# mpkuse/rgbd_odometry

Measured on NVIDIA B200. Metric: frame-pairs aligned/s (640x480, 4-lvl), higher is better.
Workload: dtype f32+f64

## Files before the change

rgbd_odometry_b200/csrc/capi.cu:

```cuda
#include <math.h>
#include <stdarg.h>
#include <stdlib.h>

#include <algorithm>
#include <new>
#include <vector>

#include "common.cuh"

static thread_local char g_err[512] = "";

void dvo_set_error(const char* fmt, ...) {
    va_list ap; va_start(ap, fmt); vsnprintf(g_err, sizeof(g_err), fmt, ap); va_end(ap);
}

static int level_dim(int dim, int level) { return (int)nearbyint((double)dim * ldexp(1.0, -level)); }

namespace {
struct StageTimer {
    dvo_ctx* c; int stage; bool on;
    StageTimer(dvo_ctx* c_, int s) : c(c_), stage(s), on(c_->timing) { if (on) cudaEventRecord(c->ev_a, c->stream); }
    ~StageTimer() {
        if (!on) return;
        cudaEventRecord(c->ev_b, c->stream); cudaEventSynchronize(c->ev_b);
        float ms = 0.f; cudaEventElapsedTime(&ms, c->ev_a, c->ev_b); c->stage_ms[stage] += ms;
    }
};
template <typename T> int dalloc(T** p, size_t n) {
    if (n == 0) { *p = nullptr; return DVO_OK; }
    cudaError_t e = cudaMalloc((void**)p, n * sizeof(T));
    if (e != cudaSuccess) { dvo_set_error("cudaMalloc(%zu bytes) failed: %s", n * sizeof(T), cudaGetErrorString(e)); return DVO_ERR_NOMEM; }
    return DVO_OK;
}
bool range_ok(dvo_ctx* c, int first, int count) { return c && first >= 0 && count >= 0 && first + count <= c->cfg.max_batch; }
int join_aux(dvo_ctx* c) {
    if (!c || !c->aux_pending) return DVO_OK;
    c->aux_pending = false;
    for (int k = 0; k < 2; ++k) DVO_CUDA(cudaStreamWaitEvent(c->stream, c->ev_aux_done[k], 0));
    return DVO_OK;
}
}

extern "C" {

const char* dvo_last_error(void) { return g_err; }

int dvo_device_count(void) {
    int n = 0;
    if (cudaGetDeviceCount(&n) != cudaSuccess) { cudaGetLastError(); return 0; }
    return n;
}

#define CREATE_CUDA(call)                                                                       \
    do {                                                                                        \
        cudaError_t e__ = (call);                                                               \
        if (e__ != cudaSuccess) {                                                               \
            dvo_set_error("%s:%d: %s -> %s", __FILE__, __LINE__, #call, cudaGetErrorString(e__)); \
            dvo_destroy(c);                                                                     \
            return DVO_ERR_CUDA;                                                                \
        }                                                                                       \
    } while (0)

int dvo_create(const dvo_config* cfg, dvo_ctx** out) {
    if (!cfg || !out) { dvo_set_error("dvo_create: null argument"); return DVO_ERR_ARG; }
    if (cfg->width < 8 || cfg->height < 8 || cfg->levels < 1 || cfg->levels > DVO_MAX_LEVELS || cfg->max_batch < 1 || cfg->max_batch > 65535 ||
        cfg->width >= DVO_EDT_INF_1D || cfg->height >= DVO_EDT_INF_1D) {
        dvo_set_error("dvo_create: bad config %dx%d levels=%d max_batch=%d", cfg->width, cfg->height, cfg->levels, cfg->max_batch);
        return DVO_ERR_ARG;
    }
    int ndev = 0;
    cudaError_t e = cudaGetDeviceCount(&ndev);
    if (e != cudaSuccess || ndev == 0) {
        dvo_set_error("dvo_create: no usable CUDA device (%s); this library has no CPU fallback", cudaGetErrorString(e));
        cudaGetLastError();
        return DVO_ERR_CUDA;
    }
    if (cfg->device < 0 || cfg->device >= ndev) { dvo_set_error("dvo_create: device %d out of range (%d devices)", cfg->device, ndev); return DVO_ERR_ARG; }
    DVO_CUDA(cudaSetDevice(cfg->device));
    if (const char* e = getenv("DVO_L2_FETCH")) { cudaDeviceSetLimit(cudaLimitMaxL2FetchGranularity, (size_t)atoi(e)); cudaGetLastError(); }
    dvo_ctx* c = new (std::nothrow) dvo_ctx();
    if (!c) return DVO_ERR_NOMEM;
    memset(c, 0, sizeof(*c));
    c->cfg = *cfg;
    PyrGeom& g = c->geom;
    g.L = cfg->levels; g.Bmax = cfg->max_batch;
    long long acc = 0; int maxP = 0;
    for (int l = 0; l < g.L; ++l) {
        g.w[l] = level_dim(cfg->width, l); g.h[l] = level_dim(cfg->height, l);
        if (g.w[l] < 2 || g.h[l] < 2) { dvo_set_error("dvo_create: level %d is %dx%d (too small)", l, g.w[l], g.h[l]); dvo_destroy(c); return DVO_ERR_ARG; }
        g.P[l] = g.w[l] * g.h[l]; g.off[l] = acc * g.Bmax; acc += g.P[l];
        if (g.P[l] > maxP) maxP = g.P[l];
    }
    g.total = acc * g.Bmax;
    long long acct = 0;
    for (int l = 0; l < g.L; ++l) {
        g.tw[l] = (g.w[l] + 3) >> 2; g.Pt[l] = g.tw[l] * ((g.h[l] + 3) >> 2) * 16;
        g.offt[l] = acct * g.Bmax; acct += g.Pt[l];
    }
    g.total_t = acct * g.Bmax;
    cudaDeviceProp prop;
    CREATE_CUDA(cudaGetDeviceProperties(&prop, cfg->device));
    c->sm_count = prop.multiProcessorCount;
    c->smem_optin = prop.sharedMemPerBlockOptin;
    c->solve_shape = (cfg->max_batch <= c->sm_count) ? 512 : 256;
    if (const char* e = getenv("DVO_SOLVE_SHAPE")) { const int v = atoi(e); if (v == 256 || v == 512) c->solve_shape = v; }
    c->texel_mode = 1;
    c->edt_band = 0;
    if (const char* e = getenv("DVO_EDT_BAND")) c->edt_band = atoi(e);
    if (const char* e = getenv("DVO_TEXEL_MODE")) c->texel_mode = atoi(e) ? 1 : 0;
    CREATE_CUDA(cudaStreamCreateWithFlags(&c->own_stream, cudaStreamNonBlocking));
    c->stream = c->own_stream;
    CREATE_CUDA(cudaStreamCreateWithFlags(&c->copy_stream, cudaStreamNonBlocking));
    for (int i = 0; i < 16; ++i) CREATE_CUDA(cudaEventCreateWithFlags(&c->ev_chunk[i], cudaEventDisableTiming));
    CREATE_CUDA(cudaEventCreateWithFlags(&c->ev_entry, cudaEventDisableTiming));
    for (int k = 0; k < 2; ++k) {
        CREATE_CUDA(cudaStreamCreateWithFlags(&c->aux[k], cudaStreamNonBlocking));
        CREATE_CUDA(cudaEventCreateWithFlags(&c->ev_pre[k], cudaEventDisableTiming));
        CREATE_CUDA(cudaEventCreateWithFlags(&c->ev_aux_done[k], cudaEventDisableTiming));
    }
    CREATE_CUDA(cudaEventCreateWithFlags(&c->ev_fork, cudaEventDisableTiming));
    c->e2e_chunk = 128;
    if (const char* e = getenv("DVO_E2E_CHUNK")) { const int v = atoi(e); if (v > 0) c->e2e_chunk = v; }
    CREATE_CUDA(cudaEventCreate(&c->ev_a));
    CREATE_CUDA(cudaEventCreate(&c->ev_b));

    const size_t T = (size_t)g.total, B = (size_t)g.Bmax;
    int rc = DVO_OK;
    auto A = [&](int r) { if (rc == DVO_OK) rc = r; };
    for (int f = 0; f < 2; ++f) { A(dalloc(&c->gray[f], T)); A(dalloc(&c->edge[f], T)); }
    A(dalloc(&c->depth[0], T));
    if (cfg->keep_now_depth) { A(dalloc(&c->depth[1], T)); A(dalloc(&c->prev_gray, B * (size_t)g.P[0])); A(dalloc(&c->prev_depth, B * (size_t)g.P[0])); }
    c->now_valid = (unsigned char*)calloc(B, 1); c->prev_valid = (unsigned char*)calloc(B, 1);
    A(dalloc(&c->gcol, T)); A(dalloc(&c->d2, T));
    if (c->texel_mode) A(dalloc(&c->tex8, (size_t)g.total_t)); else A(dalloc(&c->texel, T));
    A(dalloc(&c->ptsX, T)); A(dalloc(&c->ptsY, T)); A(dalloc(&c->ptsZ, T)); A(dalloc(&c->ptsPix, T));
    A(dalloc(&c->npts, B * g.L)); A(dalloc(&c->solve_order, B)); A(dalloc(&c->seq_mask, B)); A(dalloc(&c->seq_state, B)); A(dalloc(&c->nedge, 2 * B * g.L)); A(dalloc(&c->maxd2, B * g.L));
    A(dalloc(&c->pose0, B * 12)); A(dalloc(&c->pose, B * 12)); A(dalloc(&c->info, B));
    if (cfg->trace_iters > 0) A(dalloc(&c->trace, B * g.L * cfg->trace_iters * DVO_TRACE_DOUBLES));
    A(dalloc(&c->energy, B * g.L * DVO_ENERGY_ITERS));
    canny_scratch_layout(g, c->bm_off, c->bm_words, &c->bitmap_scratch_words);
    A(dalloc(&c->bitmap_scratch, c->bitmap_scratch_words * B * 2));
    if (rc != DVO_OK) { dvo_destroy(c); return rc; }
    CREATE_CUDA(cudaMemsetAsync(c->npts, 0, sizeof(int) * B * g.L, c->stream));
    CREATE_CUDA(cudaMemsetAsync(c->bitmap_scratch, 0, sizeof(uint32_t) * c->bitmap_scratch_words * B * 2, c->stream));
    CREATE_CUDA(cudaMemsetAsync(c->nedge, 0, sizeof(unsigned) * 2 * B * g.L, c->stream));
    CREATE_CUDA(cudaMemsetAsync(c->maxd2, 0, sizeof(unsigned) * B * g.L, c->stream));
    CREATE_CUDA(cudaMemsetAsync(c->info, 0, sizeof(dvo_pair_info) * B, c->stream));
    CREATE_CUDA(cudaMallocHost((void**)&c->h_pose, sizeof(double) * 12 * B));
    CREATE_CUDA(cudaMallocHost((void**)&c->h_info, sizeof(dvo_pair_info) * B));
    dvo_set_initial_pose(c, 0, g.Bmax, nullptr, DVO_MEM_HOST);
    CREATE_CUDA(cudaStreamSynchronize(c->stream));
    *out = c;
    return DVO_OK;
}

int dvo_destroy(dvo_ctx* c) {
    if (!c) return DVO_OK;
    cudaSetDevice(c->cfg.device);
    if (c->own_stream) cudaStreamSynchronize(c->own_stream);
    for (int f = 0; f < 2; ++f) { cudaFree(c->gray[f]); cudaFree(c->depth[f]); cudaFree(c->edge[f]); }
    cudaFree(c->gcol); cudaFree(c->d2); cudaFree(c->texel); cudaFree(c->tex8); cudaFree(c->ptsX); cudaFree(c->ptsY); cudaFree(c->ptsZ); cudaFree(c->ptsPix);
    cudaFree(c->npts); cudaFree(c->solve_order); cudaFree(c->seq_mask); cudaFree(c->seq_state); cudaFree(c->nedge); cudaFree(c->maxd2); cudaFree(c->pose0); cudaFree(c->pose); cudaFree(c->info);
    cudaFree(c->seq_rel); cudaFree(c->seq_kind); cudaFree(c->seq_reason); cudaFree(c->seq_glob); cudaFree(c->seq_cov); cudaFree(c->seq_gcov);
    cudaFree(c->cov_buf); cudaFree(c->cov_info_buf);
    for (int k = 0; k < 2; ++k) {
        cudaFree(c->seq_stage_g[k]); cudaFree(c->seq_stage_d[k]);
        if (c->seq_ev_ready[k]) cudaEventDestroy(c->seq_ev_ready[k]);
        if (c->seq_ev_free[k]) cudaEventDestroy(c->seq_ev_free[k]);
    }
    cudaFree(c->trace); cudaFree(c->energy); cudaFree(c->bitmap_scratch); cudaFree(c->prev_gray); cudaFree(c->prev_depth); cudaFree(c->raw_bgr); cudaFree(c->raw_depth);
    free(c->now_valid); free(c->prev_valid);
    if (c->h_pose) cudaFreeHost(c->h_pose);
    if (c->h_info) cudaFreeHost(c->h_info);
    if (c->ev_a) cudaEventDestroy(c->ev_a);
    if (c->ev_b) cudaEventDestroy(c->ev_b);
    if (c->own_stream) cudaStreamDestroy(c->own_stream);
    for (int k = 0; k < 2; ++k) {
        if (c->aux[k]) { cudaStreamSynchronize(c->aux[k]); cudaStreamDestroy(c->aux[k]); }
        if (c->ev_pre[k]) cudaEventDestroy(c->ev_pre[k]);
        if (c->ev_aux_done[k]) cudaEventDestroy(c->ev_aux_done[k]);
    }
    if (c->ev_fork) cudaEventDestroy(c->ev_fork);
    if (c->copy_stream) cudaStreamDestroy(c->copy_stream);
    for (int i = 0; i < 16; ++i) if (c->ev_chunk[i]) cudaEventDestroy(c->ev_chunk[i]);
    if (c->ev_entry) cudaEventDestroy(c->ev_entry);
    delete c;
    return DVO_OK;
}

int dvo_set_stream(dvo_ctx* c, void* s) {
    if (!c) return DVO_ERR_ARG;
    { int rc = join_aux(c); if (rc) return rc; }
    c->stream = s ? (cudaStream_t)s : c->own_stream;
    return DVO_OK;
}

int dvo_synchronize(dvo_ctx* c) {
    if (!c) return DVO_ERR_ARG;
    { int rc = join_aux(c); if (rc) return rc; }
    DVO_CUDA(cudaStreamSynchronize(c->stream));
    return DVO_OK;
}

int dvo_set_intrinsics(dvo_ctx* c, float fx, float fy, float cx, float cy) {
    if (!c) return DVO_ERR_ARG;
    c->K.fx = fx; c->K.fy = fy; c->K.cx = cx; c->K.cy = cy; c->haveK = true;
    return DVO_OK;
}

}

static int begin_set_frames(dvo_ctx* c, const char* who, int frame, int first, int count, bool have_gray, bool have_depth) {
    if (!range_ok(c, first, count) || (frame != DVO_FRAME_REF && frame != DVO_FRAME_NOW) || !have_gray) { dvo_set_error("%s: bad argument", who); return DVO_ERR_ARG; }
    if (frame == DVO_FRAME_REF && !have_depth) { dvo_set_error("%s: the reference frame needs depth", who); return DVO_ERR_ARG; }
    bool rotate = false;
    if (frame == DVO_FRAME_NOW && c->prev_gray) {
        if (!have_depth) { dvo_set_error("%s: a context with keep_now_depth needs the now frame's depth", who); return DVO_ERR_ARG; }
        bool any = false, all = true;
        for (int i = first; i < first + count; ++i) { any |= c->now_valid[i] != 0; all &= c->now_valid[i] != 0; }
        if (any && !all) { dvo_set_error("%s: slots [%d,%d) mix first and subsequent now frames", who, first, first + count); return DVO_ERR_STATE; }
        rotate = all && count > 0;
    }
    const size_t P0 = c->geom.P[0];
    if (rotate) {
        DVO_CUDA(cudaMemcpyAsync(c->prev_gray + P0 * first, c->gray[1] + lvl_at(c->geom, 0, first), P0 * count, cudaMemcpyDeviceToDevice, c->stream));
        DVO_CUDA(cudaMemcpyAsync(c->prev_depth + P0 * first, c->depth[1] + lvl_at(c->geom, 0, first), P0 * count * 2, cudaMemcpyDeviceToDevice, c->stream));
        for (int i = first; i < first + count; ++i) c->prev_valid[i] = 1;
    }
    if (frame == DVO_FRAME_NOW) for (int i = first; i < first + count; ++i) c->now_valid[i] = 1;
    return DVO_OK;
}

extern "C" {

int dvo_set_frames(dvo_ctx* c, int frame, int first, int count, const uint8_t* gray, const uint16_t* depth, int mem) {
    if (c) { const int jr = join_aux(c); if (jr) return jr; }
    { const int rc = begin_set_frames(c, "dvo_set_frames", frame, first, count, gray != nullptr, depth != nullptr); if (rc) return rc; }
    StageTimer t(c, DVO_STAGE_H2D);
    const size_t P0 = c->geom.P[0];
    const cudaMemcpyKind k = mem == DVO_MEM_DEVICE ? cudaMemcpyDeviceToDevice : cudaMemcpyHostToDevice;
    DVO_CUDA(cudaMemcpyAsync(c->gray[frame] + lvl_at(c->geom, 0, first), gray, P0 * count, k, c->stream));
    if (depth && c->depth[frame])
        DVO_CUDA(cudaMemcpyAsync(c->depth[frame] + lvl_at(c->geom, 0, first), depth, P0 * count * sizeof(uint16_t), k, c->stream));
    return DVO_OK;
}

int dvo_set_frames_raw(dvo_ctx* c, int frame, int first, int count, const uint8_t* bgr, const float* depth_m, int mem) {
    if (c) { const int jr = join_aux(c); if (jr) return jr; }
    { const int rc = begin_set_frames(c, "dvo_set_frames_raw", frame, first, count, bgr != nullptr, depth_m != nullptr); if (rc) return rc; }
    if (count == 0) return DVO_OK;
    StageTimer t(c, DVO_STAGE_H2D);
    const size_t P0 = c->geom.P[0];
    const uint8_t* d_bgr = bgr; const float* d_dm = depth_m;
    if (mem != DVO_MEM_DEVICE) {
        if (c->raw_capacity < (size_t)count) {
            DVO_CUDA(cudaStreamSynchronize(c->stream));
            cudaFree(c->raw_bgr); cudaFree(c->raw_depth); c->raw_bgr = nullptr; c->raw_depth = nullptr; c->raw_capacity = 0;
            int rc = dalloc(&c->raw_bgr, (size_t)count * P0 * 3); if (rc) return rc;
            rc = dalloc(&c->raw_depth, (size_t)count * P0); if (rc) return rc;
            c->raw_capacity = (size_t)count;
        }
        DVO_CUDA(cudaMemcpyAsync(c->raw_bgr, bgr, P0 * count * 3, cudaMemcpyHostToDevice, c->stream));
        if (depth_m) DVO_CUDA(cudaMemcpyAsync(c->raw_depth, depth_m, P0 * count * sizeof(float), cudaMemcpyHostToDevice, c->stream));
        d_bgr = c->raw_bgr; d_dm = depth_m ? c->raw_depth : nullptr;
    }
    return launch_ingest_raw(c, frame, first, count, d_bgr, d_dm);
}

int dvo_promote_now_to_ref(dvo_ctx* c, int first, int count) {
    if (c) { const int jr = join_aux(c); if (jr) return jr; }
    if (!range_ok(c, first, count)) return DVO_ERR_ARG;
    return launch_promote(c, first, count);
}

int dvo_build_pyramids(dvo_ctx* c, int first, int count, int frames_mask) {
    if (c) { const int jr = join_aux(c); if (jr) return jr; }
    if (!range_ok(c, first, count)) { dvo_set_error("dvo_build_pyramids: bad range"); return DVO_ERR_ARG; }
    if (count == 0) return DVO_OK;
    StageTimer t(c, DVO_STAGE_PYRAMID);
    return launch_pyramid(c, first, count, frames_mask);
}

int dvo_prepare(dvo_ctx* c, int first, int count, int frames_mask) {
    if (c) { const int jr = join_aux(c); if (jr) return jr; }
    if (!range_ok(c, first, count)) { dvo_set_error("dvo_prepare: bad range"); return DVO_ERR_ARG; }
    if (!c->haveK) { dvo_set_error("dvo_prepare: intrinsics not set (SolveDVO asserts isCameraIntrinsicsAvailable)"); return DVO_ERR_STATE; }
    if (count == 0) return DVO_OK;
    int rc;
    { StageTimer t(c, DVO_STAGE_CANNY); rc = launch_canny(c, first, count, frames_mask); if (rc) return rc; }
    if (frames_mask & 2) {
        if (c->texel_mode && c->edt_band >= 0) {
            StageTimer t(c, DVO_STAGE_EDT_ROWS); rc = launch_edt_pack(c, first, count); if (rc) return rc;
        } else {
            { StageTimer t(c, DVO_STAGE_EDT_ROWS); rc = launch_edt_rows(c, first, count); if (rc) return rc; }
            { StageTimer t(c, DVO_STAGE_NORMGRAD); rc = c->texel_mode ? launch_pack(c, first, count) : launch_normgrad(c, first, count); if (rc) return rc; }
        }
    }
    return DVO_OK;
}

int dvo_set_initial_pose(dvo_ctx* c, int first, int count, const double* R9T3, int mem) {
    if (c) { const int jr = join_aux(c); if (jr) return jr; }
    if (!range_ok(c, first, count)) return DVO_ERR_ARG;
    if (R9T3) {
        DVO_CUDA(cudaMemcpyAsync(c->pose0 + 12 * (size_t)first, R9T3, sizeof(double) * 12 * count,
                                 mem == DVO_MEM_DEVICE ? cudaMemcpyDeviceToDevice : cudaMemcpyHostToDevice, c->stream));
        if (mem != DVO_MEM_DEVICE) DVO_CUDA(cudaStreamSynchronize(c->stream));
    } else {
        std::vector<double> id((size_t)12 * count, 0.0);
        for (int i = 0; i < count; ++i) { id[12 * (size_t)i] = 1.0; id[12 * (size_t)i + 4] = 1.0; id[12 * (size_t)i + 8] = 1.0; }
        DVO_CUDA(cudaMemcpyAsync(c->pose0 + 12 * (size_t)first, id.data(), sizeof(double) * 12 * count, cudaMemcpyHostToDevice, c->stream));
        DVO_CUDA(cudaStreamSynchronize(c->stream));
    }
    return DVO_OK;
}

int dvo_run(dvo_ctx* c, int first, int count, const dvo_solver_params* p) {
    if (c) { const int jr = join_aux(c); if (jr) return jr; }
    if (!range_ok(c, first, count) || !p) { dvo_set_error("dvo_run: bad argument"); return DVO_ERR_ARG; }
    if (!c->haveK) { dvo_set_error("dvo_run: intrinsics not set"); return DVO_ERR_STATE; }
    if (count == 0) return DVO_OK;
    StageTimer t(c, DVO_STAGE_SOLVE);
    return launch_solve(c, first, count, p);
}

static int process_range(dvo_ctx* c, int first, int count, const dvo_solver_params* p, cudaEvent_t pre_done) {
    int rc;
    if ((rc = launch_pyramid(c, first, count, 3))) return rc;
    if ((rc = launch_canny(c, first, count, 3))) return rc;
    if (c->texel_mode && c->edt_band >= 0) { if ((rc = launch_edt_pack(c, first, count))) return rc; }
    else {
        if ((rc = launch_edt_rows(c, first, count))) return rc;
        if ((rc = c->texel_mode ? launch_pack(c, first, count) : launch_normgrad(c, first, count))) return rc;
    }
    if (pre_done) DVO_CUDA(cudaEventRecord(pre_done, c->stream));
    return launch_solve(c, first, count, p);
}

int dvo_process(dvo_ctx* c, int first, int count, const dvo_solver_params* p, double* d_poses) {
    if (!range_ok(c, first, count) || !p) { dvo_set_error("dvo_process: bad argument"); return DVO_ERR_ARG; }
    if (!c->haveK) { dvo_set_error("dvo_process: intrinsics not set"); return DVO_ERR_STATE; }
    if (count == 0) return DVO_OK;
    if (c->timing || count < 4 * c->sm_count) {
        int rc = join_aux(c); if (rc) return rc;
        if ((rc = dvo_build_pyramids(c, first, count, 3))) return rc;
        if ((rc = dvo_prepare(c, first, count, 3))) return rc;
        if ((rc = dvo_run(c, first, count, p))) return rc;
        if (d_poses) DVO_CUDA(cudaMemcpyAsync(d_poses, c->pose + 12 * (size_t)first, sizeof(double) * 12 * count, cudaMemcpyDeviceToDevice, c->stream));
        return DVO_OK;
    }
    if (c->aux_pending && (c->proc_first != first || c->proc_count != count)) { const int rc = join_aux(c); if (rc) return rc; }
    c->proc_first = first; c->proc_count = count;
    DVO_CUDA(cudaEventRecord(c->ev_fork, c->stream));
    const cudaStream_t user = c->stream;
    const int n0 = count / 2;
    const int starts[2] = {first, first + n0}, counts[2] = {n0, count - n0};
    int rc = DVO_OK;
    for (int k = 0; k < 2 && rc == DVO_OK; ++k) {
        cudaError_t e = cudaStreamWaitEvent(c->aux[k], c->ev_fork, 0);
        if (e == cudaSuccess && k == 1) e = cudaStreamWaitEvent(c->aux[1], c->ev_pre[0], 0);
        if (e != cudaSuccess) { dvo_set_error("dvo_process: %s", cudaGetErrorString(e)); rc = DVO_ERR_CUDA; break; }
        c->stream = c->aux[k];
        rc = process_range(c, starts[k], counts[k], p, c->ev_pre[k]);
        if (rc == DVO_OK && d_poses && cudaMemcpyAsync(d_poses + 12 * (size_t)(starts[k] - first), c->pose + 12 * (size_t)starts[k], sizeof(double) * 12 * counts[k],
                                                       cudaMemcpyDeviceToDevice, c->aux[k]) != cudaSuccess) rc = DVO_ERR_CUDA;
        if (rc == DVO_OK && cudaEventRecord(c->ev_aux_done[k], c->aux[k]) != cudaSuccess) rc = DVO_ERR_CUDA;
    }
    c->stream = user;
    c->aux_pending = true;
    if (rc != DVO_OK) join_aux(c);
    return rc;
}

int dvo_join(dvo_ctx* c) {
    if (!c) return DVO_ERR_ARG;
    return join_aux(c);
}

int dvo_join_stream(dvo_ctx* c, void* s) {
    if (!c) return DVO_ERR_ARG;
    if (!c->aux_pending) return DVO_OK;
    for (int k = 0; k < 2; ++k) DVO_CUDA(cudaStreamWaitEvent((cudaStream_t)s, c->ev_aux_done[k], 0));
    return DVO_OK;
}

int dvo_get_poses(dvo_ctx* c, int first, int count, double* R9T3, dvo_pair_info* info, int mem) {
    if (c) { const int jr = join_aux(c); if (jr) return jr; }
    if (!range_ok(c, first, count)) return DVO_ERR_ARG;
    StageTimer t(c, DVO_STAGE_D2H);
    const cudaMemcpyKind k = mem == DVO_MEM_DEVICE ? cudaMemcpyDeviceToDevice : cudaMemcpyDeviceToHost;
    if (R9T3) DVO_CUDA(cudaMemcpyAsync(R9T3, c->pose + 12 * (size_t)first, sizeof(double) * 12 * count, k, c->stream));
    if (info) DVO_CUDA(cudaMemcpyAsync(info, c->info + first, sizeof(dvo_pair_info) * count, k, c->stream));
    if (mem != DVO_MEM_DEVICE) DVO_CUDA(cudaStreamSynchronize(c->stream));
    return DVO_OK;
}

int dvo_align_batch(dvo_ctx* c, int count, const uint8_t* ref_gray, const uint16_t* ref_depth, const uint8_t* now_gray,
                    const uint16_t* now_depth, const dvo_solver_params* p, double* R9T3, dvo_pair_info* info) {
    if (c) { const int jr = join_aux(c); if (jr) return jr; }
    if (!c || count < 0 || !ref_gray || !ref_depth || !now_gray || !p) { dvo_set_error("dvo_align_batch: bad argument"); return DVO_ERR_ARG; }
    if (!c->haveK) { dvo_set_error("dvo_align_batch: intrinsics not set"); return DVO_ERR_STATE; }
    const size_t P0 = c->geom.P[0];
    const int B = c->cfg.max_batch;
    const bool timing = c->timing;
    c->timing = false;
    int rc = DVO_OK;
    for (int done = 0; done < count && rc == DVO_OK; done += B) {
        const int n = (count - done < B) ? count - done : B;
        if ((rc = dvo_set_initial_pose(c, 0, n, nullptr, DVO_MEM_HOST))) break;
        cudaError_t e = cudaEventRecord(c->ev_entry, c->stream);
        if (e == cudaSuccess) e = cudaStreamWaitEvent(c->copy_stream, c->ev_entry, 0);
        if (e != cudaSuccess) { dvo_set_error("dvo_align_batch: %s", cudaGetErrorString(e)); rc = DVO_ERR_CUDA; break; }
        int nchunks = (n + c->e2e_chunk - 1) / c->e2e_chunk;
        if (nchunks > 16) nchunks = 16;
        const int chunk = (n + nchunks - 1) / nchunks;
        int k = 0;
        for (int c0 = 0; c0 < n && rc == DVO_OK; c0 += chunk, ++k) {
            const int m = (n - c0 < chunk) ? n - c0 : chunk;
            const size_t src = P0 * (size_t)(done + c0);
            const long long dst = lvl_at(c->geom, 0, c0);
            e = cudaMemcpyAsync(c->gray[0] + dst, ref_gray + src, P0 * m, cudaMemcpyHostToDevice, c->copy_stream);
            if (e == cudaSuccess) e = cudaMemcpyAsync(c->depth[0] + dst, ref_depth + src, P0 * m * 2, cudaMemcpyHostToDevice, c->copy_stream);
            if (e == cudaSuccess) e = cudaMemcpyAsync(c->gray[1] + dst, now_gray + src, P0 * m, cudaMemcpyHostToDevice, c->copy_stream);
            if (e == cudaSuccess && now_depth && c->depth[1])
                e = cudaMemcpyAsync(c->depth[1] + dst, now_depth + src, P0 * m * 2, cudaMemcpyHostToDevice, c->copy_stream);
            if (e == cudaSuccess) e = cudaEventRecord(c->ev_chunk[k], c->copy_stream);
            if (e == cudaSuccess) e = cudaStreamWaitEvent(c->stream, c->ev_chunk[k], 0);
            if (e != cudaSuccess) { dvo_set_error("dvo_align_batch: %s", cudaGetErrorString(e)); rc = DVO_ERR_CUDA; break; }
            if ((rc = dvo_build_pyramids(c, c0, m, 3))) break;
            if ((rc = dvo_prepare(c, c0, m, 3))) break;
            if ((rc = dvo_run(c, c0, m, p))) break;
        }
        if (rc == DVO_OK)
            rc = dvo_get_poses(c, 0, n, R9T3 ? R9T3 + 12 * (size_t)done : nullptr, info ? info + done : nullptr, DVO_MEM_HOST);
    }
    c->timing = timing;
    return rc;
}

}

namespace {
__global__ void seq_gate_kernel(int nseq, int nframes, int t, dvo_keyframe_policy pol, int finest, const dvo_pair_info* __restrict__ info,
                                const double* __restrict__ pose, double* __restrict__ pose0, int* __restrict__ lastRef,
                                unsigned char* __restrict__ mask, double* __restrict__ rel, int* __restrict__ kind, int* __restrict__ reason) {
    const int s = blockIdx.x * blockDim.x + threadIdx.x;
    if (s >= nseq) return;
    const dvo_pair_info& I = info[s];
    int signal = 0, why = 0;
    if (pol.use_quality_gates) {
        if (I.laplacian_b > pol.laplacian_thresh) { signal = 1; why = 2; }
        if (I.visible_ratio[finest] < pol.visible_ratio_thresh) { signal = 1; why = 3; }
        if (I.npts[finest] < pol.min_reprojections) { signal = 1; why = 4; }
    }
    if (pol.keyframe_every > 0 && (t - lastRef[s]) == pol.keyframe_every) { signal = 1; why = 5; }
    const long long cur = (long long)s * nframes + t;
    if (signal && lastRef[s] != t - 1) {
        mask[s] = 1; lastRef[s] = t - 1;
        kind[cur - 1] = 2; reason[cur - 1] = why;
        for (int k = 0; k < 12; ++k) pose0[12 * (long long)s + k] = (k == 0 || k == 4 || k == 8) ? 1.0 : 0.0;
    } else {
        mask[s] = 0;
        for (int k = 0; k < 12; ++k) { const double v = pose[12 * (long long)s + k]; rel[12 * cur + k] = v; pose0[12 * (long long)s + k] = v; }
        kind[cur] = 0; reason[cur] = 0;
    }
}
__global__ void seq_finish_kernel(int nseq, int nframes, int t, const unsigned char* __restrict__ mask, const double* __restrict__ pose,
                                  double* __restrict__ pose0, double* __restrict__ rel, int* __restrict__ kind, int* __restrict__ reason) {
    const int s = blockIdx.x * blockDim.x + threadIdx.x;
    if (s >= nseq || !mask[s]) return;
    const long long cur = (long long)s * nframes + t;
    for (int k = 0; k < 12; ++k) { const double v = pose[12 * (long long)s + k]; rel[12 * cur + k] = v; pose0[12 * (long long)s + k] = v; }
    kind[cur] = 0; reason[cur] = 0;
}
__global__ void seq_init_kernel(int nseq, int nframes, double* __restrict__ pose0, int* __restrict__ lastRef, double* __restrict__ rel,
                                int* __restrict__ kind, int* __restrict__ reason) {
    const int s = blockIdx.x * blockDim.x + threadIdx.x;
    if (s >= nseq) return;
    lastRef[s] = 0;
    for (int k = 0; k < 12; ++k) { const double v = (k == 0 || k == 4 || k == 8) ? 1.0 : 0.0; pose0[12 * (long long)s + k] = v; rel[12 * (long long)s * nframes + k] = v; }
    kind[(long long)s * nframes] = 1; reason[(long long)s * nframes] = 1;
}

int run_sequences_core(dvo_ctx* c, int nseq, int nframes, const uint8_t* gray, const uint16_t* depth, int mem, const dvo_solver_params* p,
                       const dvo_keyframe_policy* pol, double* rel_poses, int* kind, int* reason, double* global_poses,
                       double* rel_cov, double* global_cov) {
    const char* who = rel_cov ? "dvo_run_sequences_cov" : "dvo_run_sequences";
    if (c) { const int jr = join_aux(c); if (jr) return jr; }
    if (!c || nseq < 1 || nseq > c->cfg.max_batch || nframes < 1 || !gray || !depth || !p || !pol || !rel_poses || !kind || (global_cov && !rel_cov)) {
        dvo_set_error("%s: bad argument", who); return DVO_ERR_ARG;
    }
    if (!c->prev_gray) { dvo_set_error("%s: create the context with keep_now_depth = 1", who); return DVO_ERR_STATE; }
    if (!c->haveK) { dvo_set_error("%s: intrinsics not set", who); return DVO_ERR_STATE; }
    int finest = -1;
    for (int l = 0; l < c->geom.L; ++l) if (p->iters[l] > 0) { finest = l; break; }
    if (finest < 0) { dvo_set_error("%s: no level has iterations", who); return DVO_ERR_ARG; }
    const size_t P0 = c->geom.P[0], n = (size_t)nseq * nframes;
    const bool host_in = (mem != DVO_MEM_DEVICE);
    int rc = DVO_OK;
    auto fail = [&](cudaError_t e) { if (e != cudaSuccess && rc == DVO_OK) { dvo_set_error("%s: %s", who, cudaGetErrorString(e)); rc = DVO_ERR_CUDA; } return rc != DVO_OK; };

    if (c->seq_rec_n < n) {
        cudaFree(c->seq_rel); cudaFree(c->seq_kind); cudaFree(c->seq_reason); c->seq_rel = nullptr; c->seq_kind = nullptr; c->seq_reason = nullptr; c->seq_rec_n = 0;
        fail(cudaMalloc((void**)&c->seq_rel, sizeof(double) * 12 * n)); fail(cudaMalloc((void**)&c->seq_kind, sizeof(int) * n)); fail(cudaMalloc((void**)&c->seq_reason, sizeof(int) * n));
        if (rc == DVO_OK) c->seq_rec_n = n;
    }
    if (host_in && c->seq_stage_slots < (size_t)nseq) {
        for (int k = 0; k < 2; ++k) { cudaFree(c->seq_stage_g[k]); cudaFree(c->seq_stage_d[k]); c->seq_stage_g[k] = nullptr; c->seq_stage_d[k] = nullptr; }
        c->seq_stage_slots = 0;
        for (int k = 0; k < 2 && rc == DVO_OK; ++k) {
            fail(cudaMalloc((void**)&c->seq_stage_g[k], P0 * nseq)); fail(cudaMalloc((void**)&c->seq_stage_d[k], P0 * nseq * sizeof(uint16_t)));
            if (!c->seq_ev_ready[k]) fail(cudaEventCreateWithFlags(&c->seq_ev_ready[k], cudaEventDisableTiming));
            if (!c->seq_ev_free[k]) fail(cudaEventCreateWithFlags(&c->seq_ev_free[k], cudaEventDisableTiming));
        }
        if (rc == DVO_OK) c->seq_stage_slots = (size_t)nseq;
    }
    if (rel_cov && c->seq_cov_n < n) {
        cudaFree(c->seq_cov); c->seq_cov = nullptr; c->seq_cov_n = 0;
        if (!fail(cudaMalloc((void**)&c->seq_cov, sizeof(double) * 36 * n))) c->seq_cov_n = n;
    }
    if (rc != DVO_OK) return rc;
    double* d_rel = c->seq_rel; int* d_kind = c->seq_kind; int* d_reason = c->seq_reason; double* d_glob = nullptr;
    uint8_t* stage_g[2] = {c->seq_stage_g[0], c->seq_stage_g[1]}; uint16_t* stage_d[2] = {c->seq_stage_d[0], c->seq_stage_d[1]};
    cudaEvent_t ev_ready[2] = {c->seq_ev_ready[0], c->seq_ev_ready[1]}, ev_free[2] = {c->seq_ev_free[0], c->seq_ev_free[1]};
    fail(cudaMemsetAsync(d_rel, 0, sizeof(double) * 12 * n, c->stream));
    fail(cudaMemsetAsync(d_kind, 0, sizeof(int) * n, c->stream));
    fail(cudaMemsetAsync(d_reason, 0, sizeof(int) * n, c->stream));
    if (rel_cov) fail(cudaMemsetAsync(c->seq_cov, 0, sizeof(double) * 36 * n, c->stream));
    if (host_in) { fail(cudaEventRecord(c->ev_entry, c->stream)); fail(cudaStreamWaitEvent(c->copy_stream, c->ev_entry, 0)); }

    bool staged_before[2] = {false, false};
    auto upload = [&](int t) {
        if (!host_in || t >= nframes || rc != DVO_OK) return;
        const int k = t & 1;
        if (staged_before[k]) fail(cudaStreamWaitEvent(c->copy_stream, ev_free[k], 0));
        fail(cudaMemcpy2DAsync(stage_g[k], P0, gray + (size_t)t * P0, (size_t)nframes * P0, P0, nseq, cudaMemcpyHostToDevice, c->copy_stream));
        fail(cudaMemcpy2DAsync(stage_d[k], P0 * 2, depth + (size_t)t * P0, (size_t)nframes * P0 * 2, P0 * 2, nseq, cudaMemcpyHostToDevice, c->copy_stream));
        fail(cudaEventRecord(ev_ready[k], c->copy_stream));
        staged_before[k] = true;
    };
    auto ingest = [&](int frame, int t) {
        if (rc != DVO_OK) return;
        uint8_t* dg = c->gray[frame] + lvl_at(c->geom, 0, 0); uint16_t* dd = c->depth[frame] + lvl_at(c->geom, 0, 0);
        if (frame == DVO_FRAME_NOW && c->now_valid[0]) {
            if (rc == DVO_OK) rc = launch_copy_bytes(c, c->prev_gray, dg, P0 * nseq);
            if (rc == DVO_OK) rc = launch_copy_bytes(c, c->prev_depth, dd, P0 * nseq * 2);
            for (int s2 = 0; s2 < nseq; ++s2) c->prev_valid[s2] = 1;
        }
        if (frame == DVO_FRAME_NOW) for (int s2 = 0; s2 < nseq; ++s2) c->now_valid[s2] = 1;
        if (host_in) {
            const int k = t & 1;
            fail(cudaStreamWaitEvent(c->stream, ev_ready[k], 0));
            if (rc == DVO_OK) rc = launch_copy_bytes(c, dg, stage_g[k], P0 * nseq);
            if (rc == DVO_OK) rc = launch_copy_bytes(c, dd, stage_d[k], P0 * nseq * 2);
            fail(cudaEventRecord(ev_free[k], c->stream));
        } else {
            fail(cudaMemcpy2DAsync(dg, P0, gray + (size_t)t * P0, (size_t)nframes * P0, P0, nseq, cudaMemcpyDeviceToDevice, c->stream));
            fail(cudaMemcpy2DAsync(dd, P0 * 2, depth + (size_t)t * P0, (size_t)nframes * P0 * 2, P0 * 2, nseq, cudaMemcpyDeviceToDevice, c->stream));
        }
    };

    const int blk = (nseq + 127) / 128;
    const bool timing = c->timing;
    c->timing = false;
    for (int s2 = 0; s2 < nseq; ++s2) { c->now_valid[s2] = 0; c->prev_valid[s2] = 0; }
    upload(0); upload(1);
    ingest(DVO_FRAME_REF, 0);
    if (rc == DVO_OK) rc = dvo_build_pyramids(c, 0, nseq, 1);
    if (rc == DVO_OK) rc = dvo_prepare(c, 0, nseq, 1);
    if (rc == DVO_OK) { seq_init_kernel<<<blk, 128, 0, c->stream>>>(nseq, nframes, c->pose0, c->seq_state, d_rel, d_kind, d_reason); c->launches++; fail(cudaGetLastError()); }
    int host_last_ref = 0;
    for (int t = 1; t < nframes && rc == DVO_OK; ++t) {
        ingest(DVO_FRAME_NOW, t);
        upload(t + 1);
        if (rc != DVO_OK) break;
        if ((rc = dvo_build_pyramids(c, 0, nseq, 2))) break;
        if ((rc = dvo_prepare(c, 0, nseq, 2))) break;
        bool switch_pass = t >= 2, first_solve = true;
        if (!pol->use_quality_gates) {
            switch_pass = t >= 2 && pol->keyframe_every > 0 && (t - host_last_ref) == pol->keyframe_every && host_last_ref != t - 1;
            if (switch_pass) { host_last_ref = t - 1; first_solve = false; }
        }
        if (first_solve && (rc = dvo_run(c, 0, nseq, p))) break;
        seq_gate_kernel<<<blk, 128, 0, c->stream>>>(nseq, nframes, t, *pol, finest, c->info, c->pose, c->pose0, c->seq_state, c->seq_mask, d_rel, d_kind, d_reason);
        c->launches++;
        if (fail(cudaGetLastError())) break;
        if (switch_pass) {
            c->active = c->seq_mask;
            rc = dvo_promote_now_to_ref(c, 0, nseq);
            if (rc == DVO_OK) rc = dvo_build_pyramids(c, 0, nseq, 1);
            if (rc == DVO_OK) rc = dvo_prepare(c, 0, nseq, 1);
            if (rc == DVO_OK) rc = dvo_run(c, 0, nseq, p);
            c->active = nullptr;
            if (rc != DVO_OK) break;
            seq_finish_kernel<<<blk, 128, 0, c->stream>>>(nseq, nframes, t, c->seq_mask, c->pose, c->pose0, d_rel, d_kind, d_reason);
            c->launches++;
            if (fail(cudaGetLastError())) break;
        }
        if (rel_cov && (rc = launch_cov(c, 0, nseq, finest, p, c->seq_cov + 36 * (size_t)t, nullptr, nframes))) break;
    }
    c->active = nullptr;
    c->timing = timing;
    if (rc == DVO_OK && (global_poses || global_cov)) {
        if (c->seq_glob_n < n) {
            cudaFree(c->seq_glob); c->seq_glob = nullptr; c->seq_glob_n = 0;
            if (!fail(cudaMalloc((void**)&c->seq_glob, sizeof(double) * 19 * n))) c->seq_glob_n = n;
        }
        if (global_cov && rc == DVO_OK && c->seq_gcov_n < n) {
            cudaFree(c->seq_gcov); c->seq_gcov = nullptr; c->seq_gcov_n = 0;
            if (!fail(cudaMalloc((void**)&c->seq_gcov, sizeof(double) * 36 * n))) c->seq_gcov_n = n;
        }
        d_glob = c->seq_glob;
        if (rc == DVO_OK) {
            rc = launch_gop(c, nseq, nframes, d_kind, d_rel, d_glob, global_cov ? c->seq_cov : nullptr, global_cov ? c->seq_gcov : nullptr);
            if (rc == DVO_OK && global_poses) fail(cudaMemcpyAsync(global_poses, d_glob, sizeof(double) * 19 * n, cudaMemcpyDeviceToHost, c->stream));
            if (rc == DVO_OK && global_cov) fail(cudaMemcpyAsync(global_cov, c->seq_gcov, sizeof(double) * 36 * n, cudaMemcpyDeviceToHost, c->stream));
        }
    }
    if (rc == DVO_OK) {
        fail(cudaMemcpyAsync(rel_poses, d_rel, sizeof(double) * 12 * n, cudaMemcpyDeviceToHost, c->stream));
        fail(cudaMemcpyAsync(kind, d_kind, sizeof(int) * n, cudaMemcpyDeviceToHost, c->stream));
        if (reason) fail(cudaMemcpyAsync(reason, d_reason, sizeof(int) * n, cudaMemcpyDeviceToHost, c->stream));
        if (rel_cov) fail(cudaMemcpyAsync(rel_cov, c->seq_cov, sizeof(double) * 36 * n, cudaMemcpyDeviceToHost, c->stream));
    }
    cudaStreamSynchronize(c->copy_stream);
    if (cudaStreamSynchronize(c->stream) != cudaSuccess && rc == DVO_OK) { dvo_set_error("%s: %s", who, cudaGetErrorString(cudaGetLastError())); rc = DVO_ERR_CUDA; }
    return rc;
}
}

extern "C" {

int dvo_run_sequences(dvo_ctx* c, int nseq, int nframes, const uint8_t* gray, const uint16_t* depth, const dvo_solver_params* p,
                      int keyframe_every, double* rel_poses, int* kind, double* global_poses) {
    dvo_keyframe_policy pol; memset(&pol, 0, sizeof(pol));
    pol.keyframe_every = keyframe_every; pol.use_quality_gates = 0; pol.laplacian_thresh = 3.0f; pol.visible_ratio_thresh = 0.8f; pol.min_reprojections = 50;
    return run_sequences_core(c, nseq, nframes, gray, depth, DVO_MEM_HOST, p, &pol, rel_poses, kind, nullptr, global_poses, nullptr, nullptr);
}

int dvo_run_sequences_gated(dvo_ctx* c, int nseq, int nframes, const uint8_t* gray, const uint16_t* depth, const dvo_solver_params* p,
                            const dvo_keyframe_policy* pol, double* rel_poses, int* kind, int* reason, double* global_poses) {
    return run_sequences_core(c, nseq, nframes, gray, depth, DVO_MEM_HOST, p, pol, rel_poses, kind, reason, global_poses, nullptr, nullptr);
}

int dvo_run_sequences_mem(dvo_ctx* c, int nseq, int nframes, const uint8_t* gray, const uint16_t* depth, int mem, const dvo_solver_params* p,
                          const dvo_keyframe_policy* pol, double* rel_poses, int* kind, int* reason, double* global_poses) {
    return run_sequences_core(c, nseq, nframes, gray, depth, mem, p, pol, rel_poses, kind, reason, global_poses, nullptr, nullptr);
}

int dvo_run_sequences_cov(dvo_ctx* c, int nseq, int nframes, const uint8_t* gray, const uint16_t* depth, int mem, const dvo_solver_params* p,
                          const dvo_keyframe_policy* pol, double* rel_poses, int* kind, int* reason, double* global_poses, double* rel_cov,
                          double* global_cov) {
    if (!rel_cov) { dvo_set_error("dvo_run_sequences_cov: rel_cov is required"); return DVO_ERR_ARG; }
    return run_sequences_core(c, nseq, nframes, gray, depth, mem, p, pol, rel_poses, kind, reason, global_poses, rel_cov, global_cov);
}

int dvo_pose_covariance(dvo_ctx* c, int first, int count, const dvo_solver_params* p, int level, double* cov36, dvo_cov_info* info, int mem) {
    if (c) { const int jr = join_aux(c); if (jr) return jr; }
    if (!range_ok(c, first, count) || !p || !cov36 || (mem != DVO_MEM_HOST && mem != DVO_MEM_DEVICE) || level < -1 || level >= c->geom.L ||
        (p->residual != DVO_RESIDUAL_DT_FLOOR && p->residual != DVO_RESIDUAL_DT_INTERP)) {
        dvo_set_error("dvo_pose_covariance: bad argument"); return DVO_ERR_ARG;
    }
    if (!c->haveK) { dvo_set_error("dvo_pose_covariance: intrinsics not set"); return DVO_ERR_STATE; }
    if (level < 0) for (int l = 0; l < c->geom.L; ++l) if (p->iters[l] > 0) { level = l; break; }
    if (level < 0) { dvo_set_error("dvo_pose_covariance: level = -1 and no level has iterations"); return DVO_ERR_ARG; }
    if (count == 0) return DVO_OK;
    if (mem == DVO_MEM_DEVICE) return launch_cov(c, first, count, level, p, cov36, info, 1);
    if (c->cov_cap < (size_t)count) {
        DVO_CUDA(cudaStreamSynchronize(c->stream));
        cudaFree(c->cov_buf); cudaFree(c->cov_info_buf); c->cov_buf = nullptr; c->cov_info_buf = nullptr; c->cov_cap = 0;
        int rc = dalloc(&c->cov_buf, (size_t)count * 36); if (rc) return rc;
        rc = dalloc(&c->cov_info_buf, (size_t)count); if (rc) return rc;
        c->cov_cap = (size_t)count;
    }
    const int rc = launch_cov(c, first, count, level, p, c->cov_buf, c->cov_info_buf, 1);
    if (rc) return rc;
    DVO_CUDA(cudaMemcpyAsync(cov36, c->cov_buf, sizeof(double) * 36 * count, cudaMemcpyDeviceToHost, c->stream));
    if (info) DVO_CUDA(cudaMemcpyAsync(info, c->cov_info_buf, sizeof(dvo_cov_info) * count, cudaMemcpyDeviceToHost, c->stream));
    DVO_CUDA(cudaStreamSynchronize(c->stream));
    return DVO_OK;
}

int dvo_level_dims(dvo_ctx* c, int level, int* w, int* h) {
    if (!c || level < 0 || level >= c->geom.L) return DVO_ERR_ARG;
    if (w) *w = c->geom.w[level];
    if (h) *h = c->geom.h[level];
    return DVO_OK;
}

int dvo_get_level_buffer(dvo_ctx* c, int slot, int frame, int level, int which, void* dst, size_t bytes) {
    if (c) { const int jr = join_aux(c); if (jr) return jr; }
    if (!range_ok(c, slot, 1) || level < 0 || level >= c->geom.L || (frame != 0 && frame != 1) || !dst) { dvo_set_error("dvo_get_level_buffer: bad argument"); return DVO_ERR_ARG; }
    const size_t P = c->geom.P[level];
    const long long o = lvl_at(c->geom, level, slot);
    const void* src = nullptr; size_t es = 0;
    switch (which) {
        case DVO_BUF_GRAY: src = c->gray[frame] + o; es = 1; break;
        case DVO_BUF_DEPTH: if (!c->depth[frame]) { dvo_set_error("depth not stored for this frame"); return DVO_ERR_STATE; } src = c->depth[frame] + o; es = 2; break;
        case DVO_BUF_EDGE: src = c->edge[frame] + o; es = 1; break;
        case DVO_BUF_D2: if (frame != DVO_FRAME_NOW) { dvo_set_error("d2 exists for the now frame only"); return DVO_ERR_ARG; } src = c->d2 + o; es = 4; break;
        case DVO_BUF_DTN: case DVO_BUF_GX: case DVO_BUF_GY:
            if (frame != DVO_FRAME_NOW) { dvo_set_error("DT exists for the now frame only"); return DVO_ERR_ARG; } src = c->texel ? c->texel + o : nullptr; es = 16; break;
        default: dvo_set_error("dvo_get_level_buffer: unknown buffer %d", which); return DVO_ERR_ARG;
    }
    if (which == DVO_BUF_D2 && c->texel_mode && c->edt_band >= 0) {
        if (bytes < P * 4) { dvo_set_error("dvo_get_level_buffer: destination too small"); return DVO_ERR_ARG; }
        int32_t* d_tmp = nullptr;
        DVO_CUDA(cudaMalloc((void**)&d_tmp, P * 4));
        const int rc = launch_d2_from_texels(c, slot, level, d_tmp);
        cudaError_t ce = rc ? cudaSuccess : cudaMemcpyAsync(dst, d_tmp, P * 4, cudaMemcpyDeviceToHost, c->stream);
        if (ce == cudaSuccess) ce = cudaStreamSynchronize(c->stream);
        cudaFree(d_tmp);
        if (rc) return rc;
        DVO_CUDA(ce);
        return DVO_OK;
    }
    if (which >= DVO_BUF_DTN) {
        if (bytes < P * 4) { dvo_set_error("dvo_get_level_buffer: destination too small"); return DVO_ERR_ARG; }
        std::vector<float> tmp(P * 4);
        float4* d_tmp = nullptr;
        if (!src) {
            DVO_CUDA(cudaMalloc((void**)&d_tmp, P * 16));
            const int rc = c->texel_mode ? launch_resolve_texels(c, slot, level, d_tmp) : launch_normgrad_into(c, slot, level, d_tmp);
            if (rc) { cudaFree(d_tmp); return rc; }
            src = d_tmp;
        }
        cudaError_t ce = cudaMemcpyAsync(tmp.data(), src, P * 16, cudaMemcpyDeviceToHost, c->stream);
        if (ce == cudaSuccess) ce = cudaStreamSynchronize(c->stream);
        cudaFree(d_tmp);
        DVO_CUDA(ce);
        const int comp = which - DVO_BUF_DTN;
        float* d = (float*)dst;
        for (size_t i = 0; i < P; ++i) d[i] = tmp[4 * i + comp];
        return DVO_OK;
    }
    if (bytes < P * es) { dvo_set_error("dvo_get_level_buffer: destination too small"); return DVO_ERR_ARG; }
    DVO_CUDA(cudaMemcpyAsync(dst, src, P * es, cudaMemcpyDeviceToHost, c->stream));
    DVO_CUDA(cudaStreamSynchronize(c->stream));
    if (which == DVO_BUF_DEPTH && level == 0) {
        uint16_t* d = (uint16_t*)dst;
        for (size_t i = 0; i < P; ++i) if (d[i] == 0) d[i] = 1;
    }
    return DVO_OK;
}

static int reference_order(dvo_ctx* c, int slot, int level, int n, std::vector<int>& perm) {
    perm.resize(n);
    if (n == 0) return DVO_OK;
    std::vector<int> pix(n);
    DVO_CUDA(cudaMemcpyAsync(pix.data(), c->ptsPix + lvl_at(c->geom, level, slot), sizeof(int) * n, cudaMemcpyDeviceToHost, c->stream));
    DVO_CUDA(cudaStreamSynchronize(c->stream));
    const int w = c->geom.w[level], h = c->geom.h[level];
    std::vector<long long> key(n);
    for (int i = 0; i < n; ++i) { const int y = pix[i] / w, x = pix[i] - y * w; key[i] = ((long long)x * h + y) * (long long)n + i; }
    std::sort(key.begin(), key.end());
    for (int k = 0; k < n; ++k) perm[k] = (int)(key[k] % n);
    return DVO_OK;
}

int dvo_get_points(dvo_ctx* c, int slot, int level, float* X, float* Y, float* Z, int capacity, int* n) {
    if (c) { const int jr = join_aux(c); if (jr) return jr; }
    if (!range_ok(c, slot, 1) || level < 0 || level >= c->geom.L || !n) return DVO_ERR_ARG;
    int cnt = 0;
    DVO_CUDA(cudaMemcpyAsync(&cnt, c->npts + (size_t)slot * c->geom.L + level, sizeof(int), cudaMemcpyDeviceToHost, c->stream));
    DVO_CUDA(cudaStreamSynchronize(c->stream));
    *n = cnt;
    const int m = cnt < capacity ? cnt : capacity;
    if (m <= 0 || !(X || Y || Z)) return DVO_OK;
    std::vector<int> perm;
    int rc = reference_order(c, slot, level, cnt, perm);
    if (rc) return rc;
    const long long o = lvl_at(c->geom, level, slot);
    std::vector<float> tmp(cnt);
    float* dst[3] = {X, Y, Z}; const float* src[3] = {c->ptsX + o, c->ptsY + o, c->ptsZ + o};
    for (int a = 0; a < 3; ++a) {
        if (!dst[a]) continue;
        DVO_CUDA(cudaMemcpyAsync(tmp.data(), src[a], sizeof(float) * cnt, cudaMemcpyDeviceToHost, c->stream));
        DVO_CUDA(cudaStreamSynchronize(c->stream));
        for (int k = 0; k < m; ++k) dst[a][k] = tmp[perm[k]];
    }
    return DVO_OK;
}

int dvo_eval_normal_equations(dvo_ctx* c, int slot, int level, const double* R9T3, int jacobian, int weight, int arithmetic,
                              float huber_k, double* H36, double* g6, double* sumsq, int* nvis, float* eps, float* w, float* u,
                              float* v, float* J) {
    dvo_solver_params prm;
    memset(&prm, 0, sizeof(prm));
    prm.jacobian = jacobian; prm.weight = weight; prm.arithmetic = arithmetic; prm.huber_k = huber_k;
    return dvo_eval_normal_equations_ex(c, slot, level, R9T3, &prm, H36, g6, sumsq, nvis, eps, w, u, v, J);
}

int dvo_eval_normal_equations_ex(dvo_ctx* c, int slot, int level, const double* R9T3, const dvo_solver_params* prm,
                                 double* H36, double* g6, double* sumsq, int* nvis, float* eps, float* w, float* u, float* v, float* J) {
    if (c) { const int jr = join_aux(c); if (jr) return jr; }
    if (!prm) return DVO_ERR_ARG;
    if (!range_ok(c, slot, 1) || level < 0 || level >= c->geom.L || !R9T3) return DVO_ERR_ARG;
    if (!c->haveK) { dvo_set_error("intrinsics not set"); return DVO_ERR_STATE; }
    int N = 0;
    DVO_CUDA(cudaMemcpyAsync(&N, c->npts + (size_t)slot * c->geom.L + level, sizeof(int), cudaMemcpyDeviceToHost, c->stream));
    DVO_CUDA(cudaStreamSynchronize(c->stream));
    double* d_pose = nullptr; double* d_out = nullptr; float* d_pp = nullptr;
    const bool pp = eps || w || u || v || J;
    const size_t n1 = (size_t)(N > 0 ? N : 1);
    {
        cudaError_t e = cudaMalloc((void**)&d_pose, sizeof(double) * 12);
        if (e == cudaSuccess) e = cudaMalloc((void**)&d_out, sizeof(double) * 44);
        if (e == cudaSuccess && pp) e = cudaMalloc((void**)&d_pp, sizeof(float) * n1 * 10);
        if (e == cudaSuccess) e = cudaMemcpyAsync(d_pose, R9T3, sizeof(double) * 12, cudaMemcpyHostToDevice, c->stream);
        if (e != cudaSuccess) {
            dvo_set_error("dvo_eval_normal_equations: %s", cudaGetErrorString(e));
            cudaFree(d_pose); cudaFree(d_out); cudaFree(d_pp);
            return DVO_ERR_CUDA;
        }
    }
    float *de = nullptr, *dw = nullptr, *du = nullptr, *dv = nullptr, *dJ = nullptr;
    if (pp) { de = d_pp; dw = d_pp + n1; du = d_pp + 2 * n1; dv = d_pp + 3 * n1; dJ = d_pp + 4 * n1; }
    int rc = launch_eval(c, slot, level, d_pose, prm->jacobian, prm->weight, prm->arithmetic, prm->huber_k, prm->residual, d_out, de, dw, du, dv, dJ);
    if (rc == DVO_OK) {
        double out[44];
        std::vector<float> host(pp ? n1 * 10 : 0);
        cudaError_t e = cudaMemcpyAsync(out, d_out, sizeof(out), cudaMemcpyDeviceToHost, c->stream);
        if (e == cudaSuccess && pp && N > 0) e = cudaMemcpyAsync(host.data(), d_pp, sizeof(float) * n1 * 10, cudaMemcpyDeviceToHost, c->stream);
        if (e == cudaSuccess) e = cudaStreamSynchronize(c->stream);
        if (e != cudaSuccess) { dvo_set_error("dvo_eval_normal_equations: %s", cudaGetErrorString(e)); rc = DVO_ERR_CUDA; }
        else {
            if (g6) memcpy(g6, out, sizeof(double) * 6);
            if (H36) memcpy(H36, out + 6, sizeof(double) * 36);
            if (sumsq) *sumsq = out[42];
            if (nvis) *nvis = (int)out[43];
            if (pp && N > 0) {
                std::vector<int> perm;
                rc = reference_order(c, slot, level, N, perm);
                if (rc == DVO_OK)
                    for (int k = 0; k < N; ++k) {
                        const size_t i = (size_t)perm[k];
                        if (eps) eps[k] = host[i];
                        if (w) w[k] = host[n1 + i];
                        if (u) u[k] = host[2 * n1 + i];
                        if (v) v[k] = host[3 * n1 + i];
                        if (J) for (int q = 0; q < 6; ++q) J[6 * (size_t)k + q] = host[4 * n1 + 6 * i + q];
                    }
            }
        }
    }
    cudaFree(d_pose); cudaFree(d_out); cudaFree(d_pp);
    return rc;
}

int dvo_get_trace(dvo_ctx* c, int slot, int level, double* trace) {
    if (c) { const int jr = join_aux(c); if (jr) return jr; }
    if (!range_ok(c, slot, 1) || level < 0 || level >= c->geom.L || !trace) return DVO_ERR_ARG;
    if (!c->trace) { dvo_set_error("dvo_get_trace: context created with trace_iters = 0"); return DVO_ERR_STATE; }
    const size_t n = (size_t)c->cfg.trace_iters * DVO_TRACE_DOUBLES;
    DVO_CUDA(cudaMemcpyAsync(trace, c->trace + ((size_t)slot * c->geom.L + level) * n, sizeof(double) * n, cudaMemcpyDeviceToHost, c->stream));
    DVO_CUDA(cudaStreamSynchronize(c->stream));
    return DVO_OK;
}

int dvo_get_energies(dvo_ctx* c, int slot, int level, float* energies, int capacity) {
    if (c) { const int jr = join_aux(c); if (jr) return jr; }
    if (!range_ok(c, slot, 1) || level < 0 || level >= c->geom.L || !energies || capacity < 0) return DVO_ERR_ARG;
    const int n = capacity < DVO_ENERGY_ITERS ? capacity : DVO_ENERGY_ITERS;
    if (n == 0) return DVO_OK;
    DVO_CUDA(cudaMemcpyAsync(energies, c->energy + ((size_t)slot * c->geom.L + level) * DVO_ENERGY_ITERS, sizeof(float) * n, cudaMemcpyDeviceToHost, c->stream));
    DVO_CUDA(cudaStreamSynchronize(c->stream));
    return DVO_OK;
}

int dvo_enable_timing(dvo_ctx* c, int on) {
    if (!c) return DVO_ERR_ARG;
    c->timing = on != 0;
    for (int i = 0; i < DVO_STAGE_COUNT; ++i) c->stage_ms[i] = 0.f;
    return DVO_OK;
}

int dvo_get_stage_ms(dvo_ctx* c, float* ms) {
    if (!c || !ms) return DVO_ERR_ARG;
    for (int i = 0; i < DVO_STAGE_COUNT; ++i) { ms[i] = c->stage_ms[i]; c->stage_ms[i] = 0.f; }
    return DVO_OK;
}

long long dvo_launch_count(dvo_ctx* c) { return c ? c->launches : 0; }

int dvo_gop_compose(dvo_ctx* c, int nseq, int nframes, const int* kind, const double* rel, double* out, int mem) {
    if (c) { const int jr = join_aux(c); if (jr) return jr; }
    if (!c || nseq < 1 || nframes < 1 || !kind || !rel || !out) return DVO_ERR_ARG;
    const size_t n = (size_t)nseq * nframes;
    if (mem == DVO_MEM_DEVICE) return launch_gop(c, nseq, nframes, kind, rel, out, nullptr, nullptr);
    int* d_kind = nullptr; double* d_rel = nullptr; double* d_out = nullptr;
    {
        cudaError_t e = cudaMalloc((void**)&d_kind, sizeof(int) * n);
        if (e == cudaSuccess) e = cudaMalloc((void**)&d_rel, sizeof(double) * 12 * n);
        if (e == cudaSuccess) e = cudaMalloc((void**)&d_out, sizeof(double) * 19 * n);
        if (e == cudaSuccess) e = cudaMemcpyAsync(d_kind, kind, sizeof(int) * n, cudaMemcpyHostToDevice, c->stream);
        if (e == cudaSuccess) e = cudaMemcpyAsync(d_rel, rel, sizeof(double) * 12 * n, cudaMemcpyHostToDevice, c->stream);
        if (e != cudaSuccess) {
            dvo_set_error("dvo_gop_compose: %s", cudaGetErrorString(e));
            cudaFree(d_kind); cudaFree(d_rel); cudaFree(d_out);
            return DVO_ERR_CUDA;
        }
    }
    int rc = launch_gop(c, nseq, nframes, d_kind, d_rel, d_out, nullptr, nullptr);
    if (rc == DVO_OK) {
        cudaError_t e = cudaMemcpyAsync(out, d_out, sizeof(double) * 19 * n, cudaMemcpyDeviceToHost, c->stream);
        if (e == cudaSuccess) e = cudaStreamSynchronize(c->stream);
        if (e != cudaSuccess) { dvo_set_error("dvo_gop_compose: %s", cudaGetErrorString(e)); rc = DVO_ERR_CUDA; }
    }
    cudaFree(d_kind); cudaFree(d_rel); cudaFree(d_out);
    return rc;
}

struct dvo_blob { void* d; size_t bytes; int device; };

int dvo_blob_create(size_t bytes, int device, dvo_blob** out) {
    if (!out || bytes == 0) { dvo_set_error("dvo_blob_create: bad argument"); return DVO_ERR_ARG; }
    int ndev = 0;
    if (cudaGetDeviceCount(&ndev) != cudaSuccess || ndev < 1) { cudaGetLastError(); dvo_set_error("dvo_blob_create: no usable CUDA device (there is no CPU fallback)"); return DVO_ERR_CUDA; }
    if (device < 0 || device >= ndev) { dvo_set_error("dvo_blob_create: device %d out of range", device); return DVO_ERR_ARG; }
    DVO_CUDA(cudaSetDevice(device));
    dvo_blob* b = new (std::nothrow) dvo_blob();
    if (!b) return DVO_ERR_NOMEM;
    b->bytes = bytes; b->device = device; b->d = nullptr;
    if (cudaMalloc(&b->d, bytes) != cudaSuccess) { cudaGetLastError(); delete b; dvo_set_error("dvo_blob_create: cudaMalloc(%zu) failed", bytes); return DVO_ERR_NOMEM; }
    *out = b;
    return DVO_OK;
}
int dvo_blob_upload(dvo_blob* b, const void* host_src, size_t bytes) {
    if (!b || !host_src || bytes > b->bytes) { dvo_set_error("dvo_blob_upload: bad argument"); return DVO_ERR_ARG; }
    DVO_CUDA(cudaSetDevice(b->device));
    DVO_CUDA(cudaMemcpy(b->d, host_src, bytes, cudaMemcpyHostToDevice));
    return DVO_OK;
}
int dvo_blob_download(dvo_blob* b, void* host_dst, size_t bytes) {
    if (!b || !host_dst || bytes > b->bytes) { dvo_set_error("dvo_blob_download: bad argument"); return DVO_ERR_ARG; }
    DVO_CUDA(cudaSetDevice(b->device));
    DVO_CUDA(cudaMemcpy(host_dst, b->d, bytes, cudaMemcpyDeviceToHost));
    return DVO_OK;
}
void* dvo_blob_device_ptr(dvo_blob* b) { return b ? b->d : nullptr; }
size_t dvo_blob_bytes(dvo_blob* b) { return b ? b->bytes : 0; }
int dvo_blob_destroy(dvo_blob* b) {
    if (!b) return DVO_OK;
    cudaSetDevice(b->device);
    cudaFree(b->d);
    delete b;
    return DVO_OK;
}

}
```

rgbd_odometry_b200/csrc/common.cuh:

```cuda
#pragma once
#include <cuda_runtime.h>
#include <stdint.h>
#include <stdio.h>
#include <string.h>

#include "../../include/dvo_b200.h"

#define DVO_EDT_INF_1D 16384
#define DVO_EDT_INF (1 << 28)

struct PyrGeom {
    int L, Bmax;
    int w[DVO_MAX_LEVELS], h[DVO_MAX_LEVELS], P[DVO_MAX_LEVELS];
    long long off[DVO_MAX_LEVELS];
    long long total;
    int tw[DVO_MAX_LEVELS], Pt[DVO_MAX_LEVELS];
    long long offt[DVO_MAX_LEVELS];
    long long total_t;
};
__host__ __device__ inline long long lvl_at(const PyrGeom& g, int l, int b) { return g.off[l] + (long long)b * g.P[l]; }
__host__ __device__ inline long long tex_at(const PyrGeom& g, int l, int b) { return g.offt[l] + (long long)b * g.Pt[l]; }

#define DVO_TEX_ESCAPE 0x80000000u
__host__ __device__ inline int tex_index(int x, int y, int tw) {
    return (((y >> 2) * tw + (x >> 2)) << 4) | ((y & 2) << 2) | ((x & 2) << 1) | ((y & 1) << 1) | (x & 1);
}

struct Intr { float fx, fy, cx, cy; };

#define DVO_TRACE_DOUBLES 56
#define DVO_ENERGY_ITERS 128

struct dvo_ctx {
    dvo_config cfg;
    PyrGeom geom;
    Intr K;
    bool haveK;
    cudaStream_t own_stream, stream, copy_stream;
    cudaEvent_t ev_chunk[16], ev_entry;
    cudaStream_t aux[2];
    cudaEvent_t ev_fork, ev_pre[2], ev_aux_done[2];
    bool aux_pending;
    int proc_first, proc_count;
    int e2e_chunk;
    uint8_t* seq_stage_g[2]; uint16_t* seq_stage_d[2]; size_t seq_stage_slots;
    cudaEvent_t seq_ev_ready[2], seq_ev_free[2];
    double* seq_rel; int* seq_kind; int* seq_reason; double* seq_glob; size_t seq_rec_n, seq_glob_n;
    double* seq_cov; double* seq_gcov; size_t seq_cov_n, seq_gcov_n;
    double* cov_buf; dvo_cov_info* cov_info_buf; size_t cov_cap;
    int sm_count;
    int solve_shape;
    size_t smem_optin;

    uint8_t* gray[2];
    uint16_t* depth[2];
    uint8_t* prev_gray;
    uint16_t* prev_depth;
    unsigned char* now_valid;
    unsigned char* prev_valid;
    uint8_t* edge[2];
    uint16_t* gcol;
    int32_t* d2;
    float4* texel;
    uint2* tex8;
    int edt_band;
    int texel_mode;
    float *ptsX, *ptsY, *ptsZ;
    int* ptsPix;
    int* npts;
    int* solve_order;
    unsigned char* seq_mask;
    const unsigned char* active;
    int* seq_state;
    unsigned* nedge;
    unsigned* maxd2;
    double* pose0;
    double* pose;
    dvo_pair_info* info;
    double* trace;
    float* energy;
    uint32_t* bitmap_scratch;
    size_t bitmap_scratch_words;
    long long bm_off[DVO_MAX_LEVELS];
    int bm_words[DVO_MAX_LEVELS];
    size_t canny_smem_optin;

    uint8_t* raw_bgr; float* raw_depth; size_t raw_capacity;

    double* h_pose;
    dvo_pair_info* h_info;

    bool timing;
    cudaEvent_t ev_a, ev_b;
    float stage_ms[DVO_STAGE_COUNT];
    long long launches;
};

void dvo_set_error(const char* fmt, ...);

#define DVO_CUDA(call)                                                                          \
    do {                                                                                        \
        cudaError_t e__ = (call);                                                               \
        if (e__ != cudaSuccess) {                                                               \
            dvo_set_error("%s:%d: %s -> %s", __FILE__, __LINE__, #call, cudaGetErrorString(e__)); \
            return DVO_ERR_CUDA;                                                                \
        }                                                                                       \
    } while (0)

int launch_pyramid(dvo_ctx* c, int first, int count, int frames_mask);
int launch_canny(dvo_ctx* c, int first, int count, int frames_mask);
void canny_scratch_layout(const PyrGeom& g, long long* bm_off, int* bm_words, size_t* words_per_image);
int launch_edt_rows(dvo_ctx* c, int first, int count);
int launch_normgrad(dvo_ctx* c, int first, int count);
int launch_pack(dvo_ctx* c, int first, int count);
int launch_edt_pack(dvo_ctx* c, int first, int count);
int launch_d2_from_texels(dvo_ctx* c, int slot, int level, int32_t* d_out);
int launch_normgrad_into(dvo_ctx* c, int slot, int level, float4* d_out);
int launch_resolve_texels(dvo_ctx* c, int slot, int level, float4* d_out);
int launch_solve(dvo_ctx* c, int first, int count, const dvo_solver_params* p);
int launch_eval(dvo_ctx* c, int slot, int level, const double* d_pose12, int jac, int weight, int arith, float huber_k, int residual,
                double* d_out , float* d_eps, float* d_w, float* d_u, float* d_v, float* d_J);
int launch_cov(dvo_ctx* c, int first, int count, int level, const dvo_solver_params* p, double* d_cov, dvo_cov_info* d_info, long long stride);
int launch_gop(dvo_ctx* c, int nseq, int nframes, const int* d_kind, const double* d_rel, double* d_out, const double* d_rel_cov, double* d_glob_cov);
int launch_promote(dvo_ctx* c, int first, int count);
int launch_ingest_raw(dvo_ctx* c, int frame, int first, int count, const uint8_t* d_bgr, const float* d_depth_m);
int launch_copy_bytes(dvo_ctx* c, void* dst, const void* src, size_t n);

template <int ARITH> struct Ar;
template <> struct Ar<DVO_ARITH_EXACT> {
    static __device__ __forceinline__ float mul(float a, float b) { return __fmul_rn(a, b); }
    static __device__ __forceinline__ float add(float a, float b) { return __fadd_rn(a, b); }
    static __device__ __forceinline__ float sub(float a, float b) { return __fsub_rn(a, b); }
    static __device__ __forceinline__ float div(float a, float b) { return __fdiv_rn(a, b); }
    static __device__ __forceinline__ float dot2(float a, float b, float c, float d) { return __fadd_rn(__fmul_rn(a, b), __fmul_rn(c, d)); }
    static __device__ __forceinline__ float dot3(float a, float b, float c, float d, float e, float f) {
        return __fadd_rn(__fadd_rn(__fmul_rn(a, b), __fmul_rn(c, d)), __fmul_rn(e, f));
    }
    static __device__ __forceinline__ float diff2(float a, float b, float c, float d) { return __fsub_rn(__fmul_rn(a, b), __fmul_rn(c, d)); }
    static __device__ __forceinline__ float weight_ref(float r) {
        float rr = __fmul_rn(r, r);
        return __double2float_rn(__ddiv_rn(6.0, __dadd_rn(6.0, __dmul_rn((double)rr, 4.0))));
    }
};
template <> struct Ar<DVO_ARITH_FAST> {
    static __device__ __forceinline__ float mul(float a, float b) { return a * b; }
    static __device__ __forceinline__ float add(float a, float b) { return a + b; }
    static __device__ __forceinline__ float sub(float a, float b) { return a - b; }
    static __device__ __forceinline__ float div(float a, float b) { return __fdividef(a, b); }
    static __device__ __forceinline__ float dot2(float a, float b, float c, float d) { return fmaf(c, d, a * b); }
    static __device__ __forceinline__ float dot3(float a, float b, float c, float d, float e, float f) { return fmaf(e, f, fmaf(c, d, a * b)); }
    static __device__ __forceinline__ float diff2(float a, float b, float c, float d) { return fmaf(a, b, -(c * d)); }
    static __device__ __forceinline__ float weight_ref(float r) { return __fdividef(1.5f, fmaf(r, r, 1.5f)); }
};
```

rgbd_odometry_b200/csrc/preprocess.cu:

```cuda
#include <stdlib.h>

#include "common.cuh"

struct PyrArgs {
    PyrGeom g;
    uint8_t* gray;
    uint16_t* depth;
    int first;
    int sub_total;
    int l0;
    const unsigned char* active;
};

__global__ void __launch_bounds__(256) pyramid_nearest_kernel(PyrArgs a) {
    const int b = a.first + blockIdx.y;
    if (a.active && !a.active[b]) return;
    int q = blockIdx.x * blockDim.x + threadIdx.x;
    if (q >= a.sub_total) return;
    int l = a.l0;
    while (l < a.g.L - 1 && q >= a.g.P[l]) { q -= a.g.P[l]; ++l; }
    const int w = a.g.w[l], W0 = a.g.w[0], H0 = a.g.h[0];
    const int y = q / w, x = q - y * w;
    const int sy = min(y << l, H0 - 1), sx = min(x << l, W0 - 1);
    const long long src = lvl_at(a.g, 0, b) + (long long)sy * W0 + sx;
    const long long dst = lvl_at(a.g, l, b) + q;
    a.gray[dst] = a.gray[src];
    if (a.depth) { uint16_t d = a.depth[src]; a.depth[dst] = d == 0 ? (uint16_t)1 : d; }
}

__global__ void __launch_bounds__(256) pyramid_level1_vec4_kernel(PyrArgs a) {
    const int b = a.first + blockIdx.y;
    if (a.active && !a.active[b]) return;
    const int w1 = a.g.w[1], W0 = a.g.w[0], H0 = a.g.h[0];
    const int q4 = blockIdx.x * blockDim.x + threadIdx.x;
    if (q4 * 4 >= a.g.P[1]) return;
    const int y = (q4 * 4) / w1, x = q4 * 4 - y * w1;
    const int sy = min(2 * y, H0 - 1);
    const long long src = lvl_at(a.g, 0, b) + (long long)sy * W0 + 2 * x;
    const long long dst = lvl_at(a.g, 1, b) + (long long)q4 * 4;
    const uint2 gv = *reinterpret_cast<const uint2*>(a.gray + src);
    const uint32_t gout = (gv.x & 0xFFu) | ((gv.x >> 8) & 0xFF00u) | ((gv.y & 0xFFu) << 16) | ((gv.y << 8) & 0xFF000000u);
    *reinterpret_cast<uint32_t*>(a.gray + dst) = gout;
    if (a.depth) {
        const uint4 dv = *reinterpret_cast<const uint4*>(a.depth + src);
        uint32_t d0 = dv.x & 0xFFFFu, d1 = dv.y & 0xFFFFu, d2 = dv.z & 0xFFFFu, d3 = dv.w & 0xFFFFu;
        d0 = d0 ? d0 : 1u; d1 = d1 ? d1 : 1u; d2 = d2 ? d2 : 1u; d3 = d3 ? d3 : 1u;
        *reinterpret_cast<uint2*>(a.depth + dst) = make_uint2(d0 | (d1 << 16), d2 | (d3 << 16));
    }
}

__global__ void __launch_bounds__(256) pyramid_level1_vec8_kernel(PyrArgs a) {
    const int b = a.first + blockIdx.y;
    if (a.active && !a.active[b]) return;
    const int w1 = a.g.w[1], W0 = a.g.w[0], H0 = a.g.h[0];
    const int q8 = blockIdx.x * blockDim.x + threadIdx.x;
    if (q8 * 8 >= a.g.P[1]) return;
    const int y = (q8 * 8) / w1, x = q8 * 8 - y * w1;
    const int sy = min(2 * y, H0 - 1);
    const long long src = lvl_at(a.g, 0, b) + (long long)sy * W0 + 2 * x;
    const long long dst = lvl_at(a.g, 1, b) + (long long)q8 * 8;
    const uint4 gv = *reinterpret_cast<const uint4*>(a.gray + src);
    uint4 d0, d1;
    if (a.depth) { d0 = *reinterpret_cast<const uint4*>(a.depth + src); d1 = *reinterpret_cast<const uint4*>(a.depth + src + 8); }
    auto even_bytes = [](uint32_t lo, uint32_t hi) { return __byte_perm(lo, hi, 0x6420); };
    *reinterpret_cast<uint2*>(a.gray + dst) = make_uint2(even_bytes(gv.x, gv.y), even_bytes(gv.z, gv.w));
    if (a.depth) {
        auto fix = [](uint32_t v) { v &= 0xFFFFu; return v ? v : 1u; };
        *reinterpret_cast<uint4*>(a.depth + dst) = make_uint4(fix(d0.x) | (fix(d0.y) << 16), fix(d0.z) | (fix(d0.w) << 16),
                                                              fix(d1.x) | (fix(d1.y) << 16), fix(d1.z) | (fix(d1.w) << 16));
    }
}

__global__ void __launch_bounds__(256) pyramid_nearest_vec4_kernel(PyrArgs a) {
    const int b = a.first + blockIdx.y;
    if (a.active && !a.active[b]) return;
    int q = (blockIdx.x * blockDim.x + threadIdx.x) * 4;
    if (q >= a.sub_total) return;
    int l = a.l0;
    while (l < a.g.L - 1 && q >= a.g.P[l]) { q -= a.g.P[l]; ++l; }
    const int w = a.g.w[l], W0 = a.g.w[0], H0 = a.g.h[0];
    const int y = q / w, x = q - y * w;
    const int sy = min(y << l, H0 - 1);
    const long long row = lvl_at(a.g, 0, b) + (long long)sy * W0;
    const long long dst = lvl_at(a.g, l, b) + q;
    int sx[4];
#pragma unroll
    for (int j = 0; j < 4; ++j) sx[j] = min((x + j) << l, W0 - 1);
    uint32_t gv[4];
#pragma unroll
    for (int j = 0; j < 4; ++j) gv[j] = a.gray[row + sx[j]];
    if (a.depth) {
        uint32_t dv[4];
#pragma unroll
        for (int j = 0; j < 4; ++j) { dv[j] = a.depth[row + sx[j]]; }
#pragma unroll
        for (int j = 0; j < 4; ++j) dv[j] = dv[j] ? dv[j] : 1u;
        *reinterpret_cast<uint2*>(a.depth + dst) = make_uint2(dv[0] | (dv[1] << 16), dv[2] | (dv[3] << 16));
    }
    *reinterpret_cast<uint32_t*>(a.gray + dst) = gv[0] | (gv[1] << 8) | (gv[2] << 16) | (gv[3] << 24);
}

int launch_pyramid(dvo_ctx* c, int first, int count, int frames_mask) {
    const PyrGeom& g = c->geom;
    if (g.L < 2) return DVO_OK;
    const bool vec1 = (g.w[0] == 2 * g.w[1]) && (g.w[1] % 4 == 0);
    const int l0 = vec1 ? 2 : 1;
    int sub = 0;
    bool vec_rest = true;
    for (int l = l0; l < g.L; ++l) { sub += g.P[l]; vec_rest = vec_rest && (g.w[l] % 4 == 0) && (g.off[l] % 4 == 0) && (g.P[l] % 4 == 0); }
    for (int f = 0; f < 2; ++f) {
        if (!(frames_mask & (1 << f))) continue;
        PyrArgs a; a.g = g; a.gray = c->gray[f]; a.depth = c->depth[f]; a.first = first; a.sub_total = sub; a.l0 = l0; a.active = c->active;
        if (vec1 && g.w[1] % 8 == 0 && g.off[1] % 8 == 0 && g.P[1] % 8 == 0 && g.P[0] % 16 == 0) {
            dim3 grid1((g.P[1] / 8 + 255) / 256, count);
            pyramid_level1_vec8_kernel<<<grid1, 256, 0, c->stream>>>(a);
            c->launches++;
        } else if (vec1) {
            dim3 grid1((g.P[1] / 4 + 255) / 256, count);
            pyramid_level1_vec4_kernel<<<grid1, 256, 0, c->stream>>>(a);
            c->launches++;
        }
        if (sub > 0 && vec_rest) {
            dim3 grid((sub / 4 + 255) / 256, count);
            pyramid_nearest_vec4_kernel<<<grid, 256, 0, c->stream>>>(a);
            c->launches++;
        } else if (sub > 0) {
            dim3 grid((sub + 255) / 256, count);
            pyramid_nearest_kernel<<<grid, 256, 0, c->stream>>>(a);
            c->launches++;
        }
    }
    DVO_CUDA(cudaGetLastError());
    return DVO_OK;
}

struct CannyArgs {
    const uint8_t* gray[2];
    uint8_t* edge[2];
    const uint16_t* depth;
    uint16_t* gcol;
    float *X, *Y, *Z;
    int* pix;
    int* npts;
    unsigned* nedge[2];
    int w, h, P, L;
    int frame0;
    int count;
    long long gscratch_frame_stride;
    float tmpfx, tmpfy, tmpcx, tmpcy;
    uint32_t* gscratch;
    long long gscratch_stride;
    int first;
    int bm_words;
    const unsigned char* active;
};

__device__ __forceinline__ void sobel3(const uint8_t* __restrict__ g, int w, int h, int y, int x, int& dx, int& dy) {
    const int ym = max(y - 1, 0), yp = min(y + 1, h - 1), xm = max(x - 1, 0), xp = min(x + 1, w - 1);
    const uint8_t* r0 = g + ym * w; const uint8_t* r1 = g + y * w; const uint8_t* r2 = g + yp * w;
    const int a = r0[xm], b = r0[x], c = r0[xp], d = r1[xm], f = r1[xp], p = r2[xm], q = r2[x], r = r2[xp];
    dx = (c + 2 * f + r) - (a + 2 * d + p);
    dy = (p + 2 * q + r) - (a + 2 * b + c);
}
__device__ __forceinline__ int mag_at(const uint8_t* __restrict__ g, int w, int h, int y, int x) {
    if ((unsigned)y >= (unsigned)h || (unsigned)x >= (unsigned)w) return 0;
    int dx, dy; sobel3(g, w, h, y, x, dx, dy);
    return dx * dx + dy * dy;
}

__device__ __forceinline__ uint32_t expand4(uint32_t nib) { return (((nib & 0xFu) * 0x00204081u) & 0x01010101u) * 0xFFu; }

__device__ __forceinline__ void row_sums(const uint8_t* __restrict__ grow, int w, int x, int lane, int& hs, int& hb) {
    const int v = (x < w) ? (int)grow[x] : 0;
    int l = __shfl_up_sync(0xffffffffu, v, 1), r = __shfl_down_sync(0xffffffffu, v, 1);
    if (lane == 0) l = (x > 0 && x < w) ? (int)grow[x - 1] : v;
    if (lane == 31) r = (x + 1 < w) ? (int)grow[x + 1] : v;
    if (x + 1 >= w) r = v;
    hs = r - l; hb = l + 2 * v + r;
}

#ifndef DVO_NMS_L2_AHEAD
#define DVO_NMS_L2_AHEAD 4
#endif
#ifndef DVO_NMS_MIN_BLOCKS
#define DVO_NMS_MIN_BLOCKS 2
#endif
#ifndef DVO_NMS_ROWS
#define DVO_NMS_ROWS 48
#endif
#ifndef DVO_NMS_WARPS
#define DVO_NMS_WARPS 8
#endif
constexpr int NMS_ROWS = DVO_NMS_ROWS, NMS_WARPS = DVO_NMS_WARPS;
struct NmsArgs {
    const uint8_t* gray[2];
    uint32_t* scratch;
    long long slot_stride, frame_stride;
    long long off[DVO_MAX_LEVELS];
    long long bm_off[DVO_MAX_LEVELS];
    int w[DVO_MAX_LEVELS], h[DVO_MAX_LEVELS], P[DVO_MAX_LEVELS], bm_words[DVO_MAX_LEVELS];
    int chunks[DVO_MAX_LEVELS], strips[DVO_MAX_LEVELS], task_end[DVO_MAX_LEVELS];
    int L, first, count, frame0;
    float low, high;
    const unsigned char* active;
};
struct NmsSums { float s[4], b[4], sH, bH; };
struct NmsMags { float m[4], L, R; };
struct NmsGrad { float dx[4], dy[4]; };

template <bool VEC>
__global__ void __launch_bounds__(NMS_WARPS * 32, DVO_NMS_MIN_BLOCKS) sobel_nms_kernel(NmsArgs a) {
    const int lane = threadIdx.x & 31;
    int task = blockIdx.x * NMS_WARPS + (threadIdx.x >> 5);
    int l = 0;
    while (l < a.L && task >= a.task_end[l]) ++l;
    if (l >= a.L) return;
    if (l) task -= a.task_end[l - 1];
    const int chunks = a.chunks[l], strips = a.strips[l];
    const int chunk = task % chunks, t2 = task / chunks, strip = t2 % strips, img = t2 / strips;
    const int second = (img >= a.count) ? 1 : 0;
    const int frame = second ? DVO_FRAME_NOW : a.frame0;
    const int b = a.first + img - second * a.count;
    if (a.active && !a.active[b]) return;
    const int w = a.w[l], h = a.h[l];
    const int wd = (w + 31) >> 5, pitch = wd + 2;
    const uint8_t* __restrict__ g = a.gray[frame] + a.off[l] + (long long)b * a.P[l];
    uint32_t* Cb = a.scratch + (long long)b * a.slot_stride + (long long)frame * a.frame_stride + a.bm_off[l];
    const int bmw = a.bm_words[l];
    const int c0 = chunk << 7, xb = c0 + (lane << 2);
    const int y0 = strip * NMS_ROWS, y1 = min(h, y0 + NMS_ROWS);
    const bool first_lane = (lane == 0), last_lane = (lane == 31);
    const bool halo_valid = first_lane ? (c0 > 0) : (last_lane && c0 + 128 < w);
    const bool self_left = (xb == 0), self_right = (xb + 4 >= w);
    const int hx0 = first_lane ? c0 - 2 : c0 + 128;
    const uint32_t sel_near = 0x7440u + (first_lane ? 1u : 0u), sel_far = 0x7440u + (first_lane ? 0u : 1u);
    const float lowt = (xb < w) ? a.low : 3.0e38f, high = a.high;
    const float K = 13573.0f / 32768.0f;

    const bool in_image = (xb < w);
    const uint8_t* __restrict__ gx = g + (in_image ? xb : 0);
    const uint8_t* __restrict__ gh = g + (halo_valid ? hx0 : 0);
    const unsigned roff_max = (unsigned)((h - 1) * w);
    auto load_row = [&](unsigned roff, uint32_t& wv, uint32_t& hv) {
        if (VEC) {
            wv = in_image ? *reinterpret_cast<const uint32_t*>(gx + roff) : 0u;
            hv = halo_valid ? (uint32_t)*reinterpret_cast<const uint16_t*>(gh + roff) : 0u;
        } else {
            const uint8_t* __restrict__ row = g + roff;
            wv = 0u;
#pragma unroll
            for (int j = 0; j < 4; ++j) wv |= (uint32_t)row[min(xb + j, w - 1)] << (8 * j);
            hv = halo_valid ? ((uint32_t)row[hx0] | ((uint32_t)row[min(hx0 + 1, w - 1)] << 8)) : 0u;
        }
    };
    auto byte_f = [](uint32_t wv, uint32_t sel) { return __uint_as_float(__byte_perm(wv, 0x4B000000u, sel)) - 8388608.0f; };
    auto sums = [&](uint32_t wv, uint32_t hv, NmsSums& S) {
        float v[4];
#pragma unroll
        for (int j = 0; j < 4; ++j) v[j] = byte_f(wv, 0x7440u + j);
        const float hn = byte_f(hv, sel_near), hf = byte_f(hv, sel_far);
        float lft = __shfl_up_sync(0xffffffffu, v[3], 1), rgt = __shfl_down_sync(0xffffffffu, v[0], 1);
        if (first_lane) lft = hn;
        if (last_lane) rgt = hn;
        if (self_left) lft = v[0];
        if (self_right) rgt = v[3];
        S.s[0] = v[1] - lft;  S.s[1] = v[2] - v[0]; S.s[2] = v[3] - v[1]; S.s[3] = rgt - v[2];
        S.b[0] = fmaf(2.0f, v[0], lft) + v[1];  S.b[1] = fmaf(2.0f, v[1], v[0]) + v[2];
        S.b[2] = fmaf(2.0f, v[2], v[1]) + v[3]; S.b[3] = fmaf(2.0f, v[3], v[2]) + rgt;
        const float gm1 = first_lane ? hf : v[3], gp1 = first_lane ? v[0] : hf;
        S.sH = gp1 - gm1; S.bH = fmaf(2.0f, hn, gm1) + gp1;
    };
    auto grad_mag = [&](bool inside, const NmsSums& A, const NmsSums& B, const NmsSums& Cs, NmsGrad& G, NmsMags& M) {
        float mH;
        if (inside) {
#pragma unroll
            for (int j = 0; j < 4; ++j) {
                G.dx[j] = fmaf(2.0f, B.s[j], A.s[j]) + Cs.s[j]; G.dy[j] = Cs.b[j] - A.b[j];
                M.m[j] = fmaf(G.dx[j], G.dx[j], G.dy[j] * G.dy[j]);
            }
            const float dxH = fmaf(2.0f, B.sH, A.sH) + Cs.sH, dyH = Cs.bH - A.bH;
            mH = halo_valid ? fmaf(dxH, dxH, dyH * dyH) : 0.0f;
            if (!VEC) {
#pragma unroll
                for (int j = 0; j < 4; ++j) if (xb + j >= w) M.m[j] = 0.0f;
            }
        } else {
#pragma unroll
            for (int j = 0; j < 4; ++j) { G.dx[j] = 0.0f; G.dy[j] = 0.0f; M.m[j] = 0.0f; }
            mH = 0.0f;
        }
        M.L = __shfl_up_sync(0xffffffffu, M.m[3], 1); M.R = __shfl_down_sync(0xffffffffu, M.m[0], 1);
        if (first_lane) M.L = mH;
        if (last_lane) M.R = mH;
        if (self_right) M.R = 0.0f;
    };

    uint32_t wv, hv;
    NmsSums S0, S1, S2;
    NmsMags M0, M1, M2;
    NmsGrad G0, G1;
    auto row_off = [&](int r) { return min((unsigned)max(r, 0) * (unsigned)w, roff_max); };
    load_row(row_off(y0 - 2), wv, hv); sums(wv, hv, S0);
    load_row(row_off(y0 - 1), wv, hv); sums(wv, hv, S1);
    load_row(row_off(y0), wv, hv);     sums(wv, hv, S2);
    grad_mag(y0 > 0, S0, S1, S2, G0, M0);
    load_row(row_off(y0 + 1), wv, hv); sums(wv, hv, S0);
    grad_mag(true, S1, S2, S0, G0, M1);
    uint32_t wvn, hvn;
    load_row(row_off(y0 + 2), wvn, hvn);
    unsigned roff_next = row_off(y0 + 3);
    unsigned roff_l2 = row_off(y0 + 3 + DVO_NMS_L2_AHEAD);

    const int widx = (c0 >> 5) + (lane >> 3);
    const bool writer = ((lane & 7) == 0) && widx < wd;
    uint32_t* Cp = Cb + (long long)(y0 + 1) * pitch + 1 + widx;
    const int sh = (lane & 3) << 2;

    auto nms_row = [&](const NmsMags& P, const NmsMags& C, const NmsMags& N, const NmsGrad& Gc) {
        float crm[4], ncm[4];
#pragma unroll
        for (int j = 0; j < 4; ++j) { crm[j] = ((j < 3) ? C.m[j < 3 ? j + 1 : 3] : C.R) - 0.5f; ncm[j] = N.m[j] - 0.5f; }
        uint32_t bits = 0u;
#pragma unroll
        for (int j = 0; j < 4; ++j) {
            const float m = C.m[j];
            const float cl = j ? C.m[j > 0 ? j - 1 : 0] : C.L;
            const float pl = j ? P.m[j > 0 ? j - 1 : 0] : P.L, pr = (j < 3) ? P.m[j < 3 ? j + 1 : 3] : P.R;
            const float nl = j ? N.m[j > 0 ? j - 1 : 0] : N.L, nr = (j < 3) ? N.m[j < 3 ? j + 1 : 3] : N.R;
            const float adx = fabsf(Gc.dx[j]), ady = fabsf(Gc.dy[j]);
            const float t = adx * K, u = fmaf(adx, -2.0f, ady);
            const bool horiz = ady < t, vert = u > t;
            const bool neg = Gc.dx[j] * Gc.dy[j] < 0.0f;
            const float da = neg ? pr : pl, db = neg ? nl : nr;
            const float na = horiz ? cl : (vert ? P.m[j] : da);
            const float nb = horiz ? crm[j] : (vert ? ncm[j] : db);
            const bool cand = (m > na) && (m > nb) && (m > lowt);
            const bool strong = cand && (m > high);
            bits |= (cand ? (1u << j) : 0u) | (strong ? (0x10000u << j) : 0u);
        }
        bits <<= sh;
        bits |= __shfl_xor_sync(0xffffffffu, bits, 1);
        bits |= __shfl_xor_sync(0xffffffffu, bits, 2);
        const uint32_t hi = __shfl_down_sync(0xffffffffu, bits, 4);
        if (writer) {
            Cp[0] = __byte_perm(bits, hi, 0x5410);
            Cp[bmw] = __byte_perm(bits, hi, 0x7632);
        }
        Cp += pitch;
    };
    auto row_step = [&](const NmsSums& A, const NmsSums& B, NmsSums& Cs, const NmsMags& P, const NmsMags& C, NmsMags& N,
                        const NmsGrad& Gc, NmsGrad& Gn) {
        wv = wvn; hv = hvn;
        load_row(roff_next, wvn, hvn); roff_next = min(roff_next + (unsigned)w, roff_max);
        if (DVO_NMS_L2_AHEAD > 0) {
            if (in_image) asm volatile("prefetch.global.L2 [%0];" :: "l"(gx + roff_l2));
            roff_l2 = min(roff_l2 + (unsigned)w, roff_max);
        }
        sums(wv, hv, Cs);
        grad_mag(true, A, B, Cs, Gn, N);
        nms_row(P, C, N, Gc);
    };
    const int yend = (y1 == h) ? y1 - 1 : y1;
    int y = y0;
    for (; y + 6 <= yend; y += 6) {
        row_step(S2, S0, S1, M0, M1, M2, G0, G1);
        row_step(S0, S1, S2, M1, M2, M0, G1, G0);
        row_step(S1, S2, S0, M2, M0, M1, G0, G1);
        row_step(S2, S0, S1, M0, M1, M2, G1, G0);
        row_step(S0, S1, S2, M1, M2, M0, G0, G1);
        row_step(S1, S2, S0, M2, M0, M1, G1, G0);
    }
    for (; y < yend; ++y) {
        row_step(S2, S0, S1, M0, M1, M2, G0, G1);
        S2 = S0; S0 = S1; M0 = M1; M1 = M2; G0 = G1;
    }
    if (y1 == h) {
        grad_mag(false, S2, S0, S1, G1, M2);
        nms_row(M0, M1, M2, G0);
    }
}

constexpr int CANNY_MAX_WARPS = 24;
#ifndef DVO_CANNY_INTERLEAVE
#define DVO_CANNY_INTERLEAVE 1
#endif
#ifndef DVO_CANNY_STOP_AFTER
#define DVO_CANNY_STOP_AFTER 0
#endif

template <bool GLOBAL_BITMAPS> struct HystPtr { typedef volatile uint32_t* type; };
template <> struct HystPtr<true> { typedef uint32_t* type; };

template <bool GLOBAL_BITMAPS>
__global__ void __launch_bounds__(768, 2) canny_kernel(CannyArgs a) {
    extern __shared__ uint32_t smem_u32[];
    __shared__ int s_scan[CANNY_MAX_WARPS + 1];
    __shared__ int s_base;
    __shared__ unsigned s_cnt;
    __shared__ unsigned char s_chg[2][768];
    const int T = blockDim.x;
    const int tid = threadIdx.x, lane = tid & 31, warp = tid >> 5;
#if DVO_CANNY_INTERLEAVE
    const bool both = a.count != 0x7fffffff;
    const int second = both ? (int)(blockIdx.x & 1u) : 0;
    const int frame = second ? DVO_FRAME_NOW : a.frame0;
    const int b = a.first + (both ? (int)(blockIdx.x >> 1) : (int)blockIdx.x);
#else
    const int second = (blockIdx.x >= (unsigned)a.count) ? 1 : 0;
    const int frame = second ? DVO_FRAME_NOW : a.frame0;
    const int b = a.first + (int)blockIdx.x - second * a.count;
#endif
    const bool do_points = (frame == DVO_FRAME_REF), do_cols = (frame == DVO_FRAME_NOW);
    if (a.active && !a.active[b]) return;
    const int w = a.w, h = a.h;
    const int wd = (w + 31) >> 5, pitch = wd + 2;
    const int nwords = a.bm_words;
    uint32_t* C = GLOBAL_BITMAPS ? a.gscratch + (long long)b * a.gscratch_stride + (long long)frame * a.gscratch_frame_stride : smem_u32;
    uint32_t* E = C + nwords;

    if (GLOBAL_BITMAPS) {
        for (int i = tid; i < pitch; i += T) { C[i] = 0u; E[i] = 0u; C[(h + 1) * pitch + i] = 0u; E[(h + 1) * pitch + i] = 0u; }
        for (int y = tid; y < h; y += T) {
            C[(y + 1) * pitch] = 0u; E[(y + 1) * pitch] = 0u; C[(y + 1) * pitch + wd + 1] = 0u; E[(y + 1) * pitch + wd + 1] = 0u;
        }
    } else {
        const uint32_t* __restrict__ src = a.gscratch + (long long)b * a.gscratch_stride + (long long)frame * a.gscratch_frame_stride;
        if ((reinterpret_cast<uintptr_t>(src) & 15) == 0 && (nwords & 1) == 0) {
            const uint4* s4 = reinterpret_cast<const uint4*>(src); uint4* d4 = reinterpret_cast<uint4*>(C);
            for (int i = tid; i < (nwords >> 1); i += T) d4[i] = s4[i];
        } else {
            for (int i = tid; i < 2 * nwords; i += T) C[i] = src[i];
        }
    }
    if (tid == 0) { s_cnt = 0u; s_base = 0; }
    __syncthreads();

#if DVO_CANNY_STOP_AFTER == 1
    return;
#endif
    {
        const int Hs = max(1, min(h, min(T, 768) / wd));
        const int Rh = (h + Hs - 1) / Hs;
        const int items = wd * Hs;
        const int sh = tid / wd, wx = tid - sh * wd;
        const bool owner = tid < items;
        const int ya = sh * Rh, yb = min(h, ya + Rh);
        for (int i = tid; i < 2 * 768; i += T) (&s_chg[0][0])[i] = (i < 768) ? 1 : 0;
        __syncthreads();
        int cur = 0;
        for (;;) {
            int changed = 0;
            bool active = false;
            if (owner && ya < yb) {
                for (int dsy = -1; dsy <= 1 && !active; ++dsy)
                    for (int dwx = -1; dwx <= 1; ++dwx) {
                        const int s2 = sh + dsy, w2 = wx + dwx;
                        if (s2 >= 0 && s2 < Hs && w2 >= 0 && w2 < wd && s_chg[cur][s2 * wd + w2]) { active = true; break; }
                    }
            }
            if (active) {
                auto spread = [](uint32_t l, uint32_t c, uint32_t r) { return c | (c << 1) | (c >> 1) | (l >> 31) | (r << 31); };
                auto flood = [](uint32_t f, uint32_t c) {
                    const uint32_t up = ((c + f) ^ c) & c;
                    const uint32_t cr = __brev(c), fr = __brev(f);
                    return f | up | __brev(((cr + fr) ^ cr) & cr);
                };
                typename HystPtr<GLOBAL_BITMAPS>::type Ev = E;
                const uint32_t* Cv = C;
                {
                    int idx = (ya + 1) * pitch + wx + 1;
                    uint32_t sp = spread(Ev[idx - pitch - 1], Ev[idx - pitch], Ev[idx - pitch + 1]);
                    uint32_t el = Ev[idx - 1], ec = Ev[idx], er = Ev[idx + 1];
                    for (int y = ya; y < yb; ++y, idx += pitch) {
                        const uint32_t nl = Ev[idx + pitch - 1], nc = Ev[idx + pitch], nr = Ev[idx + pitch + 1];
                        const uint32_t c = Cv[idx];
                        uint32_t f = ec;
                        if (c != 0u && ec != c) {
                            f = flood(ec | (c & (sp | spread(el, ec, er) | spread(nl, nc, nr))), c);
                            if (f != ec) { Ev[idx] = f; changed = 1; }
                        }
                        sp = spread(el, f, er); el = nl; ec = nc; er = nr;
                    }
                }
                {
                    int idx = yb * pitch + wx + 1;
                    uint32_t sp = spread(Ev[idx + pitch - 1], Ev[idx + pitch], Ev[idx + pitch + 1]);
                    uint32_t el = Ev[idx - 1], ec = Ev[idx], er = Ev[idx + 1];
                    for (int y = yb - 1; y >= ya; --y, idx -= pitch) {
                        const uint32_t nl = Ev[idx - pitch - 1], nc = Ev[idx - pitch], nr = Ev[idx - pitch + 1];
                        const uint32_t c = Cv[idx];
                        uint32_t f = ec;
                        if (c != 0u && ec != c) {
                            f = flood(ec | (c & (sp | spread(el, ec, er) | spread(nl, nc, nr))), c);
                            if (f != ec) { Ev[idx] = f; changed = 1; }
                        }
                        sp = spread(el, f, er); el = nl; ec = nc; er = nr;
                    }
                }
            }
            if (owner) s_chg[cur ^ 1][tid] = (unsigned char)changed;
            cur ^= 1;
            if (!__syncthreads_or(changed)) break;
        }
    }

#if DVO_CANNY_STOP_AFTER == 2
    return;
#endif
    const int nw = h * wd;
    {
        uint8_t* eo = a.edge[frame] + (long long)b * a.P;
        unsigned cnt = 0;
        const bool vec_ok = (w % 16 == 0) && ((reinterpret_cast<uintptr_t>(eo) & 15) == 0);
        for (int q = tid; q < nw; q += T) {
            const int y = q / wd, wx = q - y * wd;
            const uint32_t e = E[(y + 1) * pitch + wx + 1];
            cnt += __popc(e);
            const int x0 = wx << 5;
            if (vec_ok && x0 + 32 <= w) {
                uint4 v0, v1;
                v0.x = expand4(e); v0.y = expand4(e >> 4); v0.z = expand4(e >> 8); v0.w = expand4(e >> 12);
                v1.x = expand4(e >> 16); v1.y = expand4(e >> 20); v1.z = expand4(e >> 24); v1.w = expand4(e >> 28);
                uint4* dst = reinterpret_cast<uint4*>(eo + (long long)y * w + x0);
                dst[0] = v0; dst[1] = v1;
            } else {
                for (int i = 0; i < 32 && x0 + i < w; ++i) eo[(long long)y * w + x0 + i] = ((e >> i) & 1u) ? 255 : 0;
            }
        }
        for (int o = 16; o > 0; o >>= 1) cnt += __shfl_down_sync(0xffffffffu, cnt, o);
        if (lane == 0 && cnt) atomicAdd(&s_cnt, cnt);
    }

#if DVO_CANNY_STOP_AFTER == 3
    return;
#endif
    if (do_points) {
        const uint16_t* __restrict__ dep = a.depth + (long long)b * a.P;
        for (int q = tid; q < nw; q += T) {
            const int y = q / wd, wx = q - y * wd;
            const int idx = (y + 1) * pitch + wx + 1;
            uint32_t e = E[idx], sel = 0u;
            const uint16_t* __restrict__ dr = dep + (long long)y * w + (wx << 5);
            while (e) {
                const int i0 = __ffs(e) - 1; e &= e - 1;
                const int i1 = e ? __ffs(e) - 1 : i0; e &= e - 1;
                const int i2 = e ? __ffs(e) - 1 : i0; e &= e - 1;
                const int i3 = e ? __ffs(e) - 1 : i0; e &= e - 1;
                const unsigned d0 = dr[i0], d1 = dr[i1], d2 = dr[i2], d3 = dr[i3];
                sel |= (d0 > 100u ? 1u << i0 : 0u) | (d1 > 100u ? 1u << i1 : 0u) | (d2 > 100u ? 1u << i2 : 0u) | (d3 > 100u ? 1u << i3 : 0u);
            }
            E[idx] = sel;
        }
    }
    __syncthreads();
    if (tid == 0) a.nedge[frame][(long long)b * a.L] = s_cnt;

    const int hw = (h + 31) >> 5, hwp = hw | 1;
    uint32_t* Et = C;
    if (do_cols) {
        const int nwarps = T >> 5;
        for (int blk = warp; blk < hw * wd; blk += nwarps) {
            const int wy = blk / wd, wx = blk - wy * wd;
            const int y = (wy << 5) + lane;
            const uint32_t word = (y < h) ? E[(y + 1) * pitch + wx + 1] : 0u;
            uint32_t mine = 0u;
#pragma unroll
            for (int j = 0; j < 32; ++j) { const uint32_t bt = __ballot_sync(0xffffffffu, (word >> j) & 1u); if (lane == j) mine = bt; }
            Et[((wx << 5) + lane) * hwp + wy] = mine;
        }
    }
    __syncthreads();

    if (do_cols) {
        uint16_t* gc = a.gcol + (long long)b * a.P;
        const int BIG = 1 << 20;
        for (int x = tid; x < w; x += T) {
            const uint32_t* col = Et + x * hwp;
            int lastrow = -BIG;
            int nextrow = -1;
            for (int wy = 0; wy < hw; ++wy) {
                const uint32_t Wd = col[wy];
                const int base = wy << 5;
                if (nextrow < base + 32) {
                    nextrow = BIG;
                    for (int kk = wy + 1; kk < hw; ++kk) { const uint32_t vv = col[kk]; if (vv) { nextrow = (kk << 5) + __ffs(vv) - 1; break; } }
                }
                uint16_t* o = gc + (long long)base * w + x;
#pragma unroll
                for (int bt = 0; bt < 32; ++bt) {
                    if (base + bt < h) {
                        const uint32_t mle = Wd & (0xffffffffu >> (31 - bt));
                        const uint32_t mge = Wd & (0xffffffffu << bt);
                        const int dn = mle ? bt - (31 - __clz(mle)) : base + bt - lastrow;
                        const int up = mge ? (__ffs(mge) - 1) - bt : nextrow - (base + bt);
                        o[(long long)bt * w] = (uint16_t)min(min(dn, up), DVO_EDT_INF_1D);
                    }
                }
                if (Wd) lastrow = base + 31 - __clz(Wd);
            }
        }
    }

    if (do_points) {
        const uint16_t* __restrict__ dep = a.depth + (long long)b * a.P;
        float* X = a.X + (long long)b * a.P; float* Y = a.Y + (long long)b * a.P; float* Z = a.Z + (long long)b * a.P;
        int* pix = a.pix + (long long)b * a.P;
        const int per = (nw + T - 1) / T;
        const int q0 = min(nw, tid * per), q1 = min(nw, q0 + per);
        int mycnt = 0;
        for (int q = q0; q < q1; ++q) { const int y = q / wd, wx = q - y * wd; mycnt += __popc(E[(y + 1) * pitch + wx + 1]); }
        int incl = mycnt;
        for (int o = 1; o < 32; o <<= 1) { const int t = __shfl_up_sync(0xffffffffu, incl, o); if (lane >= o) incl += t; }
        if (lane == 31) s_scan[warp] = incl;
        __syncthreads();
        if (tid < 32) {
            const int nwp = T >> 5;
            const int v = (tid < nwp) ? s_scan[tid] : 0;
            int iv = v;
            for (int o = 1; o < 32; o <<= 1) { const int t = __shfl_up_sync(0xffffffffu, iv, o); if (lane >= o) iv += t; }
            if (tid < nwp) s_scan[tid] = iv - v;
            if (tid == 31) s_scan[CANNY_MAX_WARPS] = iv;
        }
        __syncthreads();
        int off = s_scan[warp] + (incl - mycnt);
        for (int q = q0; q < q1; ++q) {
            const int y = q / wd, wx = q - y * wd;
            uint32_t v = E[(y + 1) * pitch + wx + 1];
            const uint16_t* __restrict__ dr = dep + (long long)y * w;
            while (v) {
                int xs[4], n = 0;
#pragma unroll
                for (int k = 0; k < 4; ++k) {
                    if (v) { xs[k] = (wx << 5) + __ffs(v) - 1; v &= v - 1; n = k + 1; } else xs[k] = xs[0];
                }
                unsigned dv[4];
#pragma unroll
                for (int k = 0; k < 4; ++k) dv[k] = dr[xs[k]];
#pragma unroll
                for (int k = 0; k < 4; ++k) {
                    if (k < n) {
                        const int x = xs[k];
                        const float z = __fdiv_rn((float)dv[k], 1000.0f);
                        X[off + k] = __fmul_rn(__fmul_rn(z, __fsub_rn((float)x, a.tmpcx)), a.tmpfx);
                        Y[off + k] = __fmul_rn(__fmul_rn(z, __fsub_rn((float)y, a.tmpcy)), a.tmpfy);
                        Z[off + k] = z;
                        pix[off + k] = y * w + x;
                    }
                }
                off += n;
            }
        }
        if (tid == 0) a.npts[(long long)b * a.L] = s_scan[CANNY_MAX_WARPS];
    }
}

static int canny_bitmap_words(int w, int h) {
    const int wd = (w + 31) >> 5;
    const int a = (wd + 2) * (h + 2);
    const int t = (wd << 5) * (((h + 31) >> 5) | 1);
    return a > t ? a : t;
}

void canny_scratch_layout(const PyrGeom& g, long long* bm_off, int* bm_words, size_t* words_per_image) {
    long long o = 0;
    for (int l = 0; l < g.L; ++l) { bm_off[l] = o; bm_words[l] = canny_bitmap_words(g.w[l], g.h[l]); o += 2LL * ((bm_words[l] + 3) & ~3); }
    *words_per_image = (size_t)o;
}

int launch_canny(dvo_ctx* c, int first, int count, int frames_mask) {
    const PyrGeom& g = c->geom;
    if (!(frames_mask & 3)) return DVO_OK;
    if ((frames_mask & 1) && !c->depth[0]) { dvo_set_error("canny: reference depth missing"); return DVO_ERR_STATE; }
    if (!c->bitmap_scratch) { dvo_set_error("canny: bitmap scratch missing"); return DVO_ERR_STATE; }
    const bool both = (frames_mask & 3) == 3;
    const int frame0 = (frames_mask & 1) ? DVO_FRAME_REF : DVO_FRAME_NOW;
    const long long slot_stride = (long long)c->bitmap_scratch_words, frame_stride = slot_stride * g.Bmax;
    {
        NmsArgs n;
        n.gray[0] = c->gray[0]; n.gray[1] = c->gray[1];
        n.scratch = c->bitmap_scratch; n.slot_stride = slot_stride; n.frame_stride = frame_stride;
        long long tasks = 0;
        for (int l = 0; l < g.L; ++l) {
            n.off[l] = g.off[l]; n.bm_off[l] = c->bm_off[l]; n.w[l] = g.w[l]; n.h[l] = g.h[l]; n.P[l] = g.P[l]; n.bm_words[l] = c->bm_words[l];
            n.chunks[l] = (g.w[l] + 127) >> 7; n.strips[l] = (g.h[l] + NMS_ROWS - 1) / NMS_ROWS;
            tasks += (long long)n.chunks[l] * n.strips[l] * count * (both ? 2 : 1);
            if (tasks > 0x7fffffff - NMS_WARPS) { dvo_set_error("canny: too many tiles in one launch"); return DVO_ERR_ARG; }
            n.task_end[l] = (int)tasks;
        }
        n.L = g.L; n.first = first; n.count = both ? count : 0x7fffffff; n.frame0 = frame0;
        n.low = 10000.0f; n.high = 22500.0f; n.active = c->active;
        bool vec = true;
        for (int l = 0; l < g.L; ++l) vec = vec && (g.w[l] % 4 == 0) && (g.off[l] % 4 == 0) && (g.P[l] % 4 == 0);
        const unsigned grid = (unsigned)((tasks + NMS_WARPS - 1) / NMS_WARPS);
        if (vec) sobel_nms_kernel<true><<<grid, NMS_WARPS * 32, 0, c->stream>>>(n);
        else sobel_nms_kernel<false><<<grid, NMS_WARPS * 32, 0, c->stream>>>(n);
        c->launches++;
    }
    for (int l = 0; l < g.L; ++l) {
        const int words = c->bm_words[l];
        const size_t smem = (size_t)2 * words * sizeof(uint32_t);
        const bool use_global = smem + 8192 > c->smem_optin;
        const int wdl = (g.w[l] + 31) >> 5;
        int strips = (CANNY_MAX_WARPS * 32) / wdl; if (strips > g.h[l]) strips = g.h[l]; if (strips < 1) strips = 1;
        int threads = wdl * strips; if (threads < g.w[l]) threads = g.w[l];
        int warps = (threads + 31) / 32; if (warps > CANNY_MAX_WARPS) warps = CANNY_MAX_WARPS; if (warps < 4) warps = 4;
        {
            static int cap[DVO_MAX_LEVELS] = {-1};
            if (cap[0] < 0) {
                const int dflt[DVO_MAX_LEVELS] = {24, 12, 8, 4, 4, 4};
                for (int i = 0; i < DVO_MAX_LEVELS; ++i) cap[i] = dflt[i];
                if (const char* e = getenv("DVO_CANNY_WARPS")) {
                    int i = 0;
                    for (const char* q = e; *q && i < DVO_MAX_LEVELS; ++i) { cap[i] = atoi(q); while (*q && *q != ',') ++q; if (*q == ',') ++q; }
                    for (int k = 0; k < DVO_MAX_LEVELS; ++k) if (cap[k] < 4 || cap[k] > CANNY_MAX_WARPS) cap[k] = dflt[k];
                }
            }
            if (warps > cap[l]) warps = cap[l];
        }
        const int T = warps * 32;
        CannyArgs a;
        for (int f = 0; f < 2; ++f) {
            a.gray[f] = c->gray[f] + g.off[l]; a.edge[f] = c->edge[f] + g.off[l];
            a.nedge[f] = c->nedge + (size_t)f * g.Bmax * g.L + l;
        }
        a.depth = c->depth[0] ? c->depth[0] + g.off[l] : nullptr;
        a.gcol = c->gcol + g.off[l];
        a.X = c->ptsX + g.off[l]; a.Y = c->ptsY + g.off[l]; a.Z = c->ptsZ + g.off[l]; a.pix = c->ptsPix + g.off[l];
        a.npts = c->npts + l;
        a.w = g.w[l]; a.h = g.h[l]; a.P = g.P[l]; a.L = g.L;
        a.frame0 = frame0;
        a.count = both ? count : 0x7fffffff;
        const float scaleFac = (float)ldexp(1.0, -l);
        a.tmpfx = (float)(1. / (double)(scaleFac * c->K.fx));
        a.tmpfy = (float)(1. / (double)(scaleFac * c->K.fy));
        a.tmpcx = scaleFac * c->K.cx; a.tmpcy = scaleFac * c->K.cy;
        a.gscratch = c->bitmap_scratch + c->bm_off[l];
        a.gscratch_stride = slot_stride;
        a.gscratch_frame_stride = frame_stride;
        a.first = first; a.bm_words = words; a.active = c->active;
        const int nblocks = both ? 2 * count : count;
        if (use_global) canny_kernel<true><<<nblocks, T, 0, c->stream>>>(a);
        else {
            if (smem > 48 * 1024 && smem > c->canny_smem_optin) {
                DVO_CUDA(cudaFuncSetAttribute(canny_kernel<false>, cudaFuncAttributeMaxDynamicSharedMemorySize, (int)smem));
                c->canny_smem_optin = smem;
            }
            canny_kernel<false><<<nblocks, T, smem, c->stream>>>(a);
        }
        c->launches++;
    }
    DVO_CUDA(cudaGetLastError());
    return DVO_OK;
}

#define DVO_EDT_SPARSE_DIV 2048

struct EdtArgs {
    const uint16_t* gcol; int32_t* d2; unsigned* maxd2;
    int w, h, P, L, first;
};

template <int WARPS>
__global__ void __launch_bounds__(WARPS * 32) edt_rows_kernel(EdtArgs a, const unsigned* __restrict__ nedge) {
    extern __shared__ int smem_i32[];
    const int warp = threadIdx.x >> 5, lane = threadIdx.x & 31;
    const int w = a.w;
    const int row = blockIdx.x * WARPS + warp;
    const int b = a.first + blockIdx.y;
    if (row >= a.h) return;
    {
        const unsigned ne = nedge[(long long)b * a.L];
        if (ne == 0u || (unsigned long long)ne * DVO_EDT_SPARSE_DIV >= (unsigned long long)a.P) return;
    }
    const int wp = (w + 1) & ~1;
    int* dv = smem_i32 + (size_t)warp * (w + wp);
    unsigned short* gs = reinterpret_cast<unsigned short*>(dv + w);
    unsigned short* arg = gs + wp;
    const uint16_t* __restrict__ gr = a.gcol + (long long)b * a.P + (long long)row * w;
    for (int x = lane; x < w; x += 32) gs[x] = gr[x];
    __syncwarp();
    constexpr int SOLO_MAX = 6;
    int n = 1; while (n < w + 1) n <<= 1;
    for (int step = n >> 1; step >= 1; step >>= 1) {
        const int cnt = ((w / step) + 1) >> 1;
        for (int j0 = 0; j0 < cnt; j0 += 32) {
            const int j = j0 + lane;
            const bool has = j < cnt;
            int m = 0, lo = 0, hi = -1;
            if (has) {
                const int p = step * (2 * j + 1);
                m = p - 1;
                const int gm = gs[m];
                lo = (p - step >= 1) ? (int)arg[p - step - 1] : 0;
                hi = (p + step <= w) ? (int)arg[p + step - 1] : w - 1;
                lo = max(lo, m - gm); hi = min(hi, m + gm);
            }
            const bool solo = has && (hi - lo < SOLO_MAX);
            if (solo) {
                int best = 0x7fffffff, bx = lo;
                for (int xq = lo; xq <= hi; ++xq) {
                    const int dxx = m - xq, gq = gs[xq]; const int v = gq * gq + dxx * dxx;
                    if (v < best) { best = v; bx = xq; }
                }
                dv[m] = best; arg[m] = (unsigned short)bx;
            }
            unsigned longmask = __ballot_sync(0xffffffffu, has && !solo);
            while (longmask) {
                const int src = __ffs(longmask) - 1; longmask &= longmask - 1;
                const int Lo = __shfl_sync(0xffffffffu, lo, src), Hi = __shfl_sync(0xffffffffu, hi, src), M = __shfl_sync(0xffffffffu, m, src);
                int best = 0x7fffffff, bx = 0x7fffffff;
                for (int xq = Lo + lane; xq <= Hi; xq += 32) {
                    const int dxx = M - xq, gq = gs[xq]; const int v = gq * gq + dxx * dxx;
                    if (v < best) { best = v; bx = xq; }
                }
                const int vmin = __reduce_min_sync(0xffffffffu, best);
                const int xmin = __reduce_min_sync(0xffffffffu, best == vmin ? bx : 0x7fffffff);
                if (lane == 0) { dv[M] = vmin; arg[M] = (unsigned short)xmin; }
            }
        }
        __syncwarp();
    }
    int32_t* out = a.d2 + (long long)b * a.P + (long long)row * w;
    int mx = 0;
    for (int x = lane; x < w; x += 32) { const int v = dv[x]; out[x] = v; mx = max(mx, v); }
    mx = __reduce_max_sync(0xffffffffu, mx);
    if (lane == 0) atomicMax(&a.maxd2[(long long)b * a.L], (unsigned)mx);
}

constexpr int EDT16_G = 170, EDT16_PAD = 192, EDT16_BIG = 30000;
#ifndef DVO_EDT_PACKED16
#define DVO_EDT_PACKED16 1
#endif
__host__ __device__ inline int edt_window_scratch_ints(int w) { return DVO_EDT_PACKED16 ? (w + 2 * EDT16_PAD + 2) : (w + 2); }

template <typename Emit>
__device__ __forceinline__ void edt_row_window(const uint16_t* __restrict__ gr, int* g2, int w, int lane, Emit emit) {
    for (int x = lane; x < w; x += 32) { const int gv = gr[x]; g2[x] = gv * gv; }
    if (lane == 0) { g2[-1] = 0x3fffffff; g2[w] = 0x3fffffff; }
    __syncwarp();
    for (int x0 = 0; x0 < w; x0 += 32) {
        const int x = x0 + lane;
        int best = (x < w) ? g2[x] : 0;
        const int kint = min(x0, w - 32 - x0);
        const int* gc = g2 + min(x, w - 1);
        int k = 1, kk = 1;
        while (k < w) {
            if (__all_sync(0xffffffffu, kk >= best)) break;
            if (k + 3 <= kint) {
                const int a0 = min(gc[-k], gc[k]), a1 = min(gc[-k - 1], gc[k + 1]), a2 = min(gc[-k - 2], gc[k + 2]), a3 = min(gc[-k - 3], gc[k + 3]);
                const int k1 = kk + 2 * k + 1, k2 = kk + 4 * k + 4, k3 = kk + 6 * k + 9;
                best = min(min(best, a0 + kk), min(a1 + k1, min(a2 + k2, a3 + k3)));
                kk += 8 * k + 16; k += 4;
            } else {
                const int vl = g2[min(max(x - k, -1), w)], vr = g2[min(x + k, w)];
                best = min(best, min(vl, vr) + kk);
                kk += 2 * k + 1; ++k;
            }
        }
        if (x < w) emit(x, best);
    }
    __syncwarp();
}

__device__ __forceinline__ void edt16_fill_pads(unsigned short* H, int w, int lane) {
    const int n = w + 2 * EDT16_PAD;
    for (int i = lane; i < EDT16_PAD; i += 32) { H[i] = EDT16_BIG; H[EDT16_PAD + w + i] = EDT16_BIG; H[n + i] = EDT16_BIG; H[n + EDT16_PAD + w + i] = EDT16_BIG; }
    __syncwarp();
}
template <typename Emit2>
__device__ __forceinline__ bool edt_row_window16(const uint16_t* __restrict__ gr, unsigned short* H, int w, int lane, Emit2 emit2) {
    const int n = w + 2 * EDT16_PAD;
    uint32_t* A = reinterpret_cast<uint32_t*>(H);
    uint32_t* B = reinterpret_cast<uint32_t*>(H + n);
    const uint32_t* __restrict__ gr2 = reinterpret_cast<const uint32_t*>(gr);
    for (int p = lane; 2 * p < w; p += 32) {
        const uint32_t gv = gr2[p];
        const uint32_t g0 = min(gv & 0xFFFFu, (uint32_t)EDT16_G), g1 = min(gv >> 16, (uint32_t)EDT16_G);
        A[(EDT16_PAD >> 1) + p] = (g0 * g0) | ((g1 * g1) << 16);
    }
    __syncwarp();
    for (int p = lane - 1; 2 * p < w; p += 32) {
        const int i = (EDT16_PAD >> 1) + p;
        B[i] = __byte_perm(A[i], A[i + 1], 0x5432);
    }
    __syncwarp();
    bool exact = true;
    for (int x0 = 0; x0 < w; x0 += 64) {
        const int x = x0 + 2 * lane;
        const int i0 = (EDT16_PAD + min(x, w - 2)) >> 1;
        uint32_t best = (x < w) ? A[i0] : 0u;
        const uint32_t* a = A + i0;
        const uint32_t* b = B + i0;
        int k = 1;
        uint32_t kk = 0x00010001u;
        for (;;) {
            const uint32_t bmax = max(best & 0xFFFFu, best >> 16);
            if (__all_sync(0xffffffffu, (kk & 0xFFFFu) >= bmax)) break;
            const int m = k >> 1;
            const uint32_t c0 = __vminu2(b[m], b[-m - 1]), c1 = __vminu2(a[m + 1], a[-m - 1]);
            const uint32_t c2 = __vminu2(b[m + 1], b[-m - 2]), c3 = __vminu2(a[m + 2], a[-m - 2]);
            const uint32_t k1 = kk + (uint32_t)(2 * k + 1) * 0x00010001u, k2 = kk + (uint32_t)(4 * k + 4) * 0x00010001u, k3 = kk + (uint32_t)(6 * k + 9) * 0x00010001u;
            best = __viaddmin_u16x2(c0, kk, best); best = __viaddmin_u16x2(c1, k1, best);
            best = __viaddmin_u16x2(c2, k2, best); best = __viaddmin_u16x2(c3, k3, best);
            kk += (uint32_t)(8 * k + 16) * 0x00010001u; k += 4;
        }
        if (x < w) {
            emit2(x, best);
            if (max(best & 0xFFFFu, best >> 16) >= (uint32_t)(EDT16_G * EDT16_G)) exact = false;
        }
    }
    __syncwarp();
    return __all_sync(0xffffffffu, exact);
}

template <int WARPS>
__global__ void __launch_bounds__(WARPS * 32) edt_rows_window_kernel(EdtArgs a, const unsigned* __restrict__ nedge) {
    extern __shared__ int smem_i32[];
    const int warp = threadIdx.x >> 5, lane = threadIdx.x & 31;
    const int w = a.w;
    const int row = blockIdx.x * WARPS + warp;
    const int b = a.first + blockIdx.y;
    if (row >= a.h) return;
    const unsigned ne = nedge[(long long)b * a.L];
    if (ne != 0u && (unsigned long long)ne * DVO_EDT_SPARSE_DIV < (unsigned long long)a.P) return;
    int32_t* out = a.d2 + (long long)b * a.P + (long long)row * w;
    if (ne == 0u) {
        for (int x = lane; x < w; x += 32) out[x] = DVO_EDT_INF;
        if (lane == 0) atomicMax(&a.maxd2[(long long)b * a.L], (unsigned)DVO_EDT_INF);
        return;
    }
    int* scratch = smem_i32 + (size_t)warp * edt_window_scratch_ints(w);
    const uint16_t* __restrict__ gr = a.gcol + (long long)b * a.P + (long long)row * w;
    int mx = 0;
    auto emit = [&](int x, int v) { out[x] = v; mx = max(mx, v); };
    const bool packed16 = DVO_EDT_PACKED16 && (w % 2 == 0) && ((reinterpret_cast<uintptr_t>(gr) & 3) == 0) && ((reinterpret_cast<uintptr_t>(out) & 7) == 0);
    bool done = false;
    if (packed16) {
        edt16_fill_pads(reinterpret_cast<unsigned short*>(scratch), w, lane);
        auto emit2 = [&](int x, uint32_t v2) {
            *reinterpret_cast<int2*>(out + x) = make_int2((int)(v2 & 0xFFFFu), (int)(v2 >> 16));
            mx = max(mx, (int)max(v2 & 0xFFFFu, v2 >> 16));
        };
        done = edt_row_window16(gr, reinterpret_cast<unsigned short*>(scratch), w, lane, emit2);
    }
    if (!done) edt_row_window(gr, scratch + 1, w, lane, emit);
    mx = __reduce_max_sync(0xffffffffu, mx);
    if (lane == 0) atomicMax(&a.maxd2[(long long)b * a.L], (unsigned)mx);
}

int launch_edt_rows(dvo_ctx* c, int first, int count) {
    const PyrGeom& g = c->geom;
    constexpr int WARPS = 8;
    DVO_CUDA(cudaMemsetAsync(c->maxd2 + (size_t)first * g.L, 0, sizeof(unsigned) * (size_t)count * g.L, c->stream));
    for (int l = 0; l < g.L; ++l) {
        EdtArgs a; a.gcol = c->gcol + g.off[l]; a.d2 = c->d2 + g.off[l]; a.maxd2 = c->maxd2 + l;
        a.w = g.w[l]; a.h = g.h[l]; a.P = g.P[l]; a.L = g.L; a.first = first;
        const unsigned* ne = c->nedge + (size_t)DVO_FRAME_NOW * g.Bmax * g.L + l;
        const int w = g.w[l];
        dim3 grid((g.h[l] + WARPS - 1) / WARPS, count);
        {
            const size_t smem = (size_t)WARPS * edt_window_scratch_ints(w) * sizeof(int);
            static size_t opted_w = 0;
            if (smem > 48 * 1024 && smem > opted_w) { DVO_CUDA(cudaFuncSetAttribute(edt_rows_window_kernel<WARPS>, cudaFuncAttributeMaxDynamicSharedMemorySize, (int)smem)); opted_w = smem; }
            edt_rows_window_kernel<WARPS><<<grid, WARPS * 32, smem, c->stream>>>(a, ne);
            c->launches++;
        }
        {
            const int wp = (w + 1) & ~1;
            const size_t smem = (size_t)WARPS * (w + wp) * sizeof(int);
            static size_t opted_b = 0;
            if (smem > 48 * 1024 && smem > opted_b) { DVO_CUDA(cudaFuncSetAttribute(edt_rows_kernel<WARPS>, cudaFuncAttributeMaxDynamicSharedMemorySize, (int)smem)); opted_b = smem; }
            edt_rows_kernel<WARPS><<<grid, WARPS * 32, smem, c->stream>>>(a, ne);
            c->launches++;
        }
    }
    DVO_CUDA(cudaGetLastError());
    return DVO_OK;
}

struct NormArgs { const int32_t* d2; float4* texel; const unsigned* maxd2; const unsigned* nedge; int w, h, P, L, first; long long out_stride; };

__global__ void __launch_bounds__(256) normgrad_kernel(NormArgs a) {
    __shared__ float tile[34][35];
    __shared__ float s_scale;
    const int b = a.first + blockIdx.z;
    const int w = a.w, h = a.h;
    const int x0 = blockIdx.x * 32, y0 = blockIdx.y * 32;
    if (threadIdx.x == 0) {
        const unsigned mx2 = a.maxd2[(long long)b * a.L];
        const unsigned ne = a.nedge[(long long)b * a.L];
        float scale = 0.0f;
        if (ne > 0u) {
            const double smax = (double)__fsqrt_rn((float)mx2);
            const double sc = 255.0 * ((smax > 2.220446049250313e-16) ? __ddiv_rn(1.0, smax) : 0.0);
            scale = __double2float_rn(sc);
        }
        s_scale = scale;
    }
    __syncthreads();
    const float scale = s_scale;
    const int32_t* __restrict__ d = a.d2 + (long long)b * a.P;
    for (int i = threadIdx.x; i < 34 * 34; i += 256) {
        const int ty = i / 34, tx = i - ty * 34;
        const int y = y0 + ty - 1, x = x0 + tx - 1;
        float v = 0.0f;
        if (x >= 0 && x < w && y >= 0 && y < h) v = __fmul_rn(__fsqrt_rn((float)__ldg(d + y * w + x)), scale);
        tile[ty][tx] = v;
    }
    __syncthreads();
    const int tx = threadIdx.x & 31;
    const int x = x0 + tx;
    if (x >= w) return;
    float4* __restrict__ out = a.texel + (long long)b * a.out_stride;
    for (int ty = threadIdx.x >> 5; ty < 32; ty += 8) {
        const int y = y0 + ty;
        if (y >= h) break;
        float4 t;
        t.x = tile[ty + 1][tx + 1];
        t.y = (x == 0 || x == w - 1) ? 0.0f : __fadd_rn(__fmul_rn(-0.5f, tile[ty + 1][tx]), __fmul_rn(0.5f, tile[ty + 1][tx + 2]));
        t.z = (y == 0 || y == h - 1) ? 0.0f : __fadd_rn(__fmul_rn(-0.5f, tile[ty][tx + 1]), __fmul_rn(0.5f, tile[ty + 2][tx + 1]));
        t.w = Ar<DVO_ARITH_EXACT>::weight_ref(t.x);
        out[(long long)y * w + x] = t;
    }
}

int launch_normgrad(dvo_ctx* c, int first, int count) {
    const PyrGeom& g = c->geom;
    for (int l = 0; l < g.L; ++l) {
        NormArgs a; a.d2 = c->d2 + g.off[l]; a.texel = c->texel + g.off[l]; a.maxd2 = c->maxd2 + l;
        a.nedge = c->nedge + (size_t)DVO_FRAME_NOW * g.Bmax * g.L + l;
        a.w = g.w[l]; a.h = g.h[l]; a.P = g.P[l]; a.L = g.L; a.first = first; a.out_stride = g.P[l];
        for (int z0 = 0; z0 < count; z0 += 32768) {
            NormArgs az = a; az.first = first + z0;
            const int nz = (count - z0 < 32768) ? count - z0 : 32768;
            dim3 grid((g.w[l] + 31) / 32, (g.h[l] + 31) / 32, nz);
            normgrad_kernel<<<grid, 256, 0, c->stream>>>(az);
            c->launches++;
        }
    }
    DVO_CUDA(cudaGetLastError());
    return DVO_OK;
}

int launch_normgrad_into(dvo_ctx* c, int slot, int level, float4* d_out) {
    const PyrGeom& g = c->geom;
    const int l = level;
    NormArgs a; a.d2 = c->d2 + g.off[l]; a.texel = d_out; a.maxd2 = c->maxd2 + l;
    a.nedge = c->nedge + (size_t)DVO_FRAME_NOW * g.Bmax * g.L + l;
    a.w = g.w[l]; a.h = g.h[l]; a.P = g.P[l]; a.L = g.L; a.first = slot; a.out_stride = 0;
    dim3 grid((g.w[l] + 31) / 32, (g.h[l] + 31) / 32, 1);
    normgrad_kernel<<<grid, 256, 0, c->stream>>>(a);
    c->launches++;
    DVO_CUDA(cudaGetLastError());
    return DVO_OK;
}

struct PackArgs { const int32_t* d2; uint2* tex8; int w, h, P, Pt, tw, th, first; };

#ifndef DVO_PACK_RH
#define DVO_PACK_RH 32
#endif
constexpr int PACK_RW = 64, PACK_RH = DVO_PACK_RH;
__global__ void __launch_bounds__(256) pack_texel_kernel(PackArgs a) {
    __shared__ int tile[PACK_RH + 2][PACK_RW + 2 + 1];
    const int b = a.first + blockIdx.z;
    const int w = a.w, h = a.h;
    const int x0 = blockIdx.x * PACK_RW, y0 = blockIdx.y * PACK_RH;
    const int32_t* __restrict__ d = a.d2 + (long long)b * a.P;
    for (int i = threadIdx.x; i < (PACK_RH + 2) * (PACK_RW + 2); i += 256) {
        const int ry = i / (PACK_RW + 2), rx = i - ry * (PACK_RW + 2);
        const int y = y0 + ry - 1, x = x0 + rx - 1;
        tile[ry][rx] = (x >= 0 && x < w && y >= 0 && y < h) ? __ldg(d + (long long)y * w + x) : 0;
    }
    __syncthreads();
    uint2* __restrict__ out = a.tex8 + (long long)b * a.Pt;
#pragma unroll
    for (int r = 0; r < PACK_RH / 4; ++r) {
        const int ty = blockIdx.y * (PACK_RH / 4) + r, tx = blockIdx.x * (PACK_RW / 4) + (threadIdx.x >> 4);
        if (ty >= a.th || tx >= a.tw) continue;
        const int k = threadIdx.x & 15;
        const int ly = (r << 2) | ((k >> 2) & 2) | ((k >> 1) & 1), lx = ((threadIdx.x >> 4) << 2) | ((k >> 1) & 2) | (k & 1);
        const int y = y0 + ly, x = x0 + lx;
        uint2 t = make_uint2(DVO_TEX_ESCAPE, 0u);
        if (x < w && y < h) {
            const int c = tile[ly + 1][lx + 1];
            const bool bx = (x == 0 || x == w - 1), by = (y == 0 || y == h - 1);
            const int dl = bx ? 0 : tile[ly + 1][lx] - c, dr = bx ? 0 : tile[ly + 1][lx + 2] - c;
            const int du = by ? 0 : tile[ly][lx + 1] - c, dd = by ? 0 : tile[ly + 2][lx + 1] - c;
            const int lo = min(min(dl, dr), min(du, dd)), hi = max(max(dl, dr), max(du, dd));
            if (c < 65536 && lo >= -512 && hi <= 511) {
                t.x = (unsigned)c | (((unsigned)dl & 0x3FFu) << 16);
                t.y = ((unsigned)dr & 0x3FFu) | (((unsigned)du & 0x3FFu) << 10) | (((unsigned)dd & 0x3FFu) << 20);
            }
        }
        out[(((long long)ty * a.tw + tx) << 4) + k] = t;
    }
}

int launch_pack(dvo_ctx* c, int first, int count) {
    const PyrGeom& g = c->geom;
    for (int l = 0; l < g.L; ++l) {
        PackArgs a; a.d2 = c->d2 + g.off[l]; a.tex8 = c->tex8 + g.offt[l];
        a.w = g.w[l]; a.h = g.h[l]; a.P = g.P[l]; a.Pt = g.Pt[l]; a.tw = g.tw[l]; a.th = (g.h[l] + 3) >> 2;
        for (int z0 = 0; z0 < count; z0 += 32768) {
            a.first = first + z0;
            const int nz = (count - z0 < 32768) ? count - z0 : 32768;
            dim3 grid((a.tw + PACK_RW / 4 - 1) / (PACK_RW / 4), (a.th + PACK_RH / 4 - 1) / (PACK_RH / 4), nz);
            pack_texel_kernel<<<grid, 256, 0, c->stream>>>(a);
            c->launches++;
        }
    }
    DVO_CUDA(cudaGetLastError());
    return DVO_OK;
}

#define DVO_D2_SPILL 64000

struct EdtPackArgs { const uint16_t* gcol; int32_t* d2; uint2* tex8; unsigned* maxd2; int w, h, P, Pt, tw, th, L, first; };

template <typename Emit>
__device__ __forceinline__ void edt_row_bisect(const uint16_t* __restrict__ gr, int* dv, unsigned short* gs, unsigned short* arg, int w, int lane, Emit emit) {
    for (int x = lane; x < w; x += 32) gs[x] = gr[x];
    __syncwarp();
    constexpr int SOLO_MAX = 6;
    int n = 1; while (n < w + 1) n <<= 1;
    for (int step = n >> 1; step >= 1; step >>= 1) {
        const int cnt = ((w / step) + 1) >> 1;
        for (int j0 = 0; j0 < cnt; j0 += 32) {
            const int j = j0 + lane;
            const bool has = j < cnt;
            int m = 0, lo = 0, hi = -1;
            if (has) {
                const int p = step * (2 * j + 1);
                m = p - 1;
                const int gm = gs[m];
                lo = (p - step >= 1) ? (int)arg[p - step - 1] : 0;
                hi = (p + step <= w) ? (int)arg[p + step - 1] : w - 1;
                lo = max(lo, m - gm); hi = min(hi, m + gm);
            }
            const bool solo = has && (hi - lo < SOLO_MAX);
            if (solo) {
                int best = 0x7fffffff, bx = lo;
                for (int xq = lo; xq <= hi; ++xq) {
                    const int dxx = m - xq, gq = gs[xq]; const int v = gq * gq + dxx * dxx;
                    if (v < best) { best = v; bx = xq; }
                }
                dv[m] = best; arg[m] = (unsigned short)bx;
            }
            unsigned longmask = __ballot_sync(0xffffffffu, has && !solo);
            while (longmask) {
                const int src = __ffs(longmask) - 1; longmask &= longmask - 1;
                const int Lo = __shfl_sync(0xffffffffu, lo, src), Hi = __shfl_sync(0xffffffffu, hi, src), M = __shfl_sync(0xffffffffu, m, src);
                int best = 0x7fffffff, bx = 0x7fffffff;
                for (int xq = Lo + lane; xq <= Hi; xq += 32) {
                    const int dxx = M - xq, gq = gs[xq]; const int v = gq * gq + dxx * dxx;
                    if (v < best) { best = v; bx = xq; }
                }
                const int vmin = __reduce_min_sync(0xffffffffu, best);
                const int xmin = __reduce_min_sync(0xffffffffu, best == vmin ? bx : 0x7fffffff);
                if (lane == 0) { dv[M] = vmin; arg[M] = (unsigned short)xmin; }
            }
        }
        __syncwarp();
    }
    for (int x = lane; x < w; x += 32) emit(x, dv[x]);
    __syncwarp();
}

template <int WARPS, int R, bool SPARSE>
__global__ void __launch_bounds__(WARPS * 32) edt_pack_kernel(EdtPackArgs a, const unsigned* __restrict__ nedge) {
    extern __shared__ int smem_i32[];
    static_assert(R % 4 == 0, "a band is a whole number of tile rows");
    const int warp = threadIdx.x >> 5, lane = threadIdx.x & 31;
    const int w = a.w, h = a.h;
    const int b = a.first + blockIdx.y;
    const unsigned ne = nedge[(long long)b * a.L];
    const bool sparse = (ne != 0u) && ((unsigned long long)ne * DVO_EDT_SPARSE_DIV < (unsigned long long)a.P);
    if (sparse != SPARSE) return;
    const int y0 = blockIdx.x * R;
    const int bp = (w + 1) & ~1;
    unsigned short* band = reinterpret_cast<unsigned short*>(smem_i32);
    const int per_warp = SPARSE ? (w + bp) : edt_window_scratch_ints(w);
    int* scratch = smem_i32 + ((R + 2) * bp) / 2 + warp * per_warp;
    int32_t* __restrict__ d2g = a.d2 + (long long)b * a.P;
    int mx = 0;
    const bool packed16 = !SPARSE && DVO_EDT_PACKED16 && (w % 2 == 0) && ne != 0u &&
                          ((reinterpret_cast<uintptr_t>(a.gcol + (long long)b * a.P) & 3) == 0);
    __shared__ int s_next_row;
    if (threadIdx.x == 0) s_next_row = WARPS;
    if (ne != 0u) {
        const int ya = max(y0 - 1, 0), yb = min(y0 + R + 1, h);
        const char* base = reinterpret_cast<const char*>(a.gcol + (long long)b * a.P + (long long)ya * w);
        const int nbytes = (yb - ya) * w * 2;
        for (int o = threadIdx.x * 128; o < nbytes; o += WARPS * 32 * 128) asm volatile("prefetch.global.L2 [%0];" :: "l"(base + o));
    }
    if (packed16) edt16_fill_pads(reinterpret_cast<unsigned short*>(scratch), w, lane);
    __syncthreads();
    for (int r = warp; r < R + 2; ) {
        const int rcur = r;
        if (lane == 0) r = atomicAdd(&s_next_row, 1);
        r = __shfl_sync(0xffffffffu, r, 0);
        const int y = y0 - 1 + rcur;
        if (y < 0 || y >= h) continue;
        unsigned short* brow = band + rcur * bp;
        int32_t* grow = d2g + (long long)y * w;
        auto emit = [&](int x, int v) {
            brow[x] = (unsigned short)min(v, 65535);
            if (v >= DVO_D2_SPILL) grow[x] = v;
            mx = max(mx, v);
        };
        if (ne == 0u) {
            for (int x = lane; x < w; x += 32) emit(x, DVO_EDT_INF);
            continue;
        }
        const uint16_t* __restrict__ gr = a.gcol + (long long)b * a.P + (long long)y * w;
        if (SPARSE) {
            unsigned short* gs = reinterpret_cast<unsigned short*>(scratch + w);
            edt_row_bisect(gr, scratch, gs, gs + bp, w, lane, emit);
        } else if (packed16) {
            unsigned* brow2 = reinterpret_cast<unsigned*>(brow);
            auto emit2 = [&](int x, uint32_t v2) { brow2[x >> 1] = v2; mx = max(mx, (int)max(v2 & 0xFFFFu, v2 >> 16)); };
            if (!edt_row_window16(gr, reinterpret_cast<unsigned short*>(scratch), w, lane, emit2)) {
                edt_row_window(gr, scratch + 1, w, lane, emit);
                edt16_fill_pads(reinterpret_cast<unsigned short*>(scratch), w, lane);
            }
        } else {
            edt_row_window(gr, scratch + 1, w, lane, emit);
        }
    }
    mx = __reduce_max_sync(0xffffffffu, mx);
    if (lane == 0 && mx > 0) atomicMax(&a.maxd2[(long long)b * a.L], (unsigned)mx);
    __syncthreads();
    uint2* __restrict__ out = a.tex8 + (long long)b * a.Pt;
    const int row_quads = a.tw << 2;
#pragma unroll 1
    for (int tyl = 0; tyl < R / 4; ++tyl) {
        const int ty = (y0 >> 2) + tyl;
        if (ty >= a.th) break;
        for (int q = threadIdx.x; q < row_quads; q += WARPS * 32) {
            const int tx = q >> 2, sub = q & 3;
            const int x = (tx << 2) | ((sub & 1) << 1), ly = (tyl << 2) | (sub & 2), y = y0 + ly;
            uint2 t[4];
#pragma unroll
            for (int k = 0; k < 4; ++k) t[k] = make_uint2(DVO_TEX_ESCAPE, 0u);
            if (x < w && y < h) {
                const unsigned short* br = band + (ly + 1) * bp + x;
                int v[4][4];
                const bool has_r = (x + 1 < w), has_b = (y + 1 < h);
#pragma unroll
                for (int r = 0; r < 4; ++r) {
                    const unsigned short* p = br + (r - 1) * bp;
                    const unsigned pr = *reinterpret_cast<const unsigned*>(p);
                    v[r][1] = (int)(pr & 0xFFFFu); v[r][2] = (int)(pr >> 16);
                    if (r == 1 || r == 2) { v[r][0] = (x > 0) ? (int)p[-1] : 0; v[r][3] = (x + 2 < w) ? (int)p[2] : 0; }
                    else { v[r][0] = 0; v[r][3] = 0; }
                }
#pragma unroll
                for (int k = 0; k < 4; ++k) {
                    const int dy = k >> 1, dx = k & 1;
                    const int px = x + dx, py = y + dy;
                    if ((dx && !has_r) || (dy && !has_b)) continue;
                    const int c = v[1 + dy][1 + dx];
                    const bool bx = (px == 0 || px == w - 1), by = (py == 0 || py == h - 1);
                    const int l = bx ? c : v[1 + dy][dx], r = bx ? c : v[1 + dy][2 + dx], u = by ? c : v[dy][1 + dx], d = by ? c : v[2 + dy][1 + dx];
                    const int dl = l - c, dr = r - c, du = u - c, dd = d - c;
                    const int lo = min(min(dl, dr), min(du, dd)), hi = max(max(dl, dr), max(du, dd));
                    if (max(max(max(c, l), max(r, u)), d) < 65535 && lo >= -512 && hi <= 511) {
                        t[k].x = (unsigned)c | (((unsigned)dl & 0x3FFu) << 16);
                        t[k].y = ((unsigned)dr & 0x3FFu) | (((unsigned)du & 0x3FFu) << 10) | (((unsigned)dd & 0x3FFu) << 20);
                    }
                }
            }
            uint4* o = reinterpret_cast<uint4*>(out + (long long)ty * (row_quads << 2) + ((long long)q << 2));
            o[0] = make_uint4(t[0].x, t[0].y, t[1].x, t[1].y);
            o[1] = make_uint4(t[2].x, t[2].y, t[3].x, t[3].y);
        }
    }
}

static size_t edt_pack_smem(int warps, int R, int w, bool sparse) {
    const int bp = (w + 1) & ~1;
    return (size_t)(R + 2) * bp * sizeof(unsigned short) + (size_t)warps * (sparse ? (w + bp) : edt_window_scratch_ints(w)) * sizeof(int);
}

template <int WARPS, int R>
static int launch_edt_pack_t(dvo_ctx* c, int first, int count) {
    const PyrGeom& g = c->geom;
    if (edt_pack_smem(WARPS, R, g.w[0], true) > c->smem_optin) {
        const int rc = launch_edt_rows(c, first, count);
        return rc ? rc : launch_pack(c, first, count);
    }
    DVO_CUDA(cudaMemsetAsync(c->maxd2 + (size_t)first * g.L, 0, sizeof(unsigned) * (size_t)count * g.L, c->stream));
    for (int l = 0; l < g.L; ++l) {
        EdtPackArgs a; a.gcol = c->gcol + g.off[l]; a.d2 = c->d2 + g.off[l]; a.tex8 = c->tex8 + g.offt[l]; a.maxd2 = c->maxd2 + l;
        a.w = g.w[l]; a.h = g.h[l]; a.P = g.P[l]; a.Pt = g.Pt[l]; a.tw = g.tw[l]; a.th = (g.h[l] + 3) >> 2; a.L = g.L; a.first = first;
        const unsigned* ne = c->nedge + (size_t)DVO_FRAME_NOW * g.Bmax * g.L + l;
        const int w = g.w[l], bp = (w + 1) & ~1;
        dim3 grid((g.h[l] + R - 1) / R, count);
        const size_t band = (size_t)(R + 2) * bp * sizeof(unsigned short);
        const size_t smem_d = band + (size_t)WARPS * edt_window_scratch_ints(w) * sizeof(int), smem_s = band + (size_t)WARPS * (w + bp) * sizeof(int);
        static size_t opted_d = 0, opted_s = 0;
        if (smem_d > 48 * 1024 && smem_d > opted_d) { DVO_CUDA(cudaFuncSetAttribute(edt_pack_kernel<WARPS, R, false>, cudaFuncAttributeMaxDynamicSharedMemorySize, (int)smem_d)); opted_d = smem_d; }
        if (smem_s > 48 * 1024 && smem_s > opted_s) { DVO_CUDA(cudaFuncSetAttribute(edt_pack_kernel<WARPS, R, true>, cudaFuncAttributeMaxDynamicSharedMemorySize, (int)smem_s)); opted_s = smem_s; }
        edt_pack_kernel<WARPS, R, false><<<grid, WARPS * 32, smem_d, c->stream>>>(a, ne);
        edt_pack_kernel<WARPS, R, true><<<grid, WARPS * 32, smem_s, c->stream>>>(a, ne);
        c->launches += 2;
    }
    DVO_CUDA(cudaGetLastError());
    return DVO_OK;
}

int launch_edt_pack(dvo_ctx* c, int first, int count) {
    const int shape = c->edt_band ? c->edt_band : (c->geom.w[0] > 800 ? -1 : 20);
    if (shape < 0) { const int rc = launch_edt_rows(c, first, count); return rc ? rc : launch_pack(c, first, count); }
    if (shape == 12) return launch_edt_pack_t<7, 12>(c, first, count);
    if (shape == 20) return launch_edt_pack_t<11, 20>(c, first, count);
    if (shape == 24) return launch_edt_pack_t<13, 24>(c, first, count);
    if (shape == 200) return launch_edt_pack_t<22, 20>(c, first, count);
    if (shape == 160) return launch_edt_pack_t<9, 16>(c, first, count);
    return launch_edt_pack_t<10, 28>(c, first, count);
}

__global__ void __launch_bounds__(256) d2_from_texels_kernel(const uint2* __restrict__ tex8, const int32_t* __restrict__ d2g, int32_t* __restrict__ out, int w, int h, int tw) {
    const int i = blockIdx.x * 256 + threadIdx.x;
    if (i >= w * h) return;
    const int y = i / w, x = i - y * w;
    const unsigned w0 = tex8[tex_index(x, y, tw)].x;
    out[i] = ((int)w0 < 0) ? d2g[i] : (int)(w0 & 0xFFFFu);
}

int launch_d2_from_texels(dvo_ctx* c, int slot, int level, int32_t* d_out) {
    const PyrGeom& g = c->geom;
    d2_from_texels_kernel<<<(g.P[level] + 255) / 256, 256, 0, c->stream>>>(c->tex8 + tex_at(g, level, slot), c->d2 + lvl_at(g, level, slot), d_out,
                                                                         g.w[level], g.h[level], g.tw[level]);
    c->launches++;
    DVO_CUDA(cudaGetLastError());
    return DVO_OK;
}

__global__ void __launch_bounds__(256) promote_masked_kernel(PyrGeom g, const uint8_t* __restrict__ prev_gray, const uint16_t* __restrict__ prev_depth,
                                                             uint8_t* __restrict__ gray, uint16_t* __restrict__ depth, int first,
                                                             const unsigned char* __restrict__ active) {
    const int b = first + blockIdx.y;
    if (!active[b]) return;
    const int P0 = g.P[0];
    const int q = (blockIdx.x * blockDim.x + threadIdx.x) * 4;
    const long long src = (long long)P0 * b, dst = lvl_at(g, 0, b);
    for (int k = q; k < min(q + 4, P0); ++k) { gray[dst + k] = prev_gray[src + k]; depth[dst + k] = prev_depth[src + k]; }
}

int launch_promote(dvo_ctx* c, int first, int count) {
    const PyrGeom& g = c->geom;
    if (!c->prev_gray) { dvo_set_error("promote: context was created without keep_now_depth"); return DVO_ERR_STATE; }
    for (int i = first; i < first + count; ++i)
        if (!c->prev_valid[i]) { dvo_set_error("promote: slot %d has no previous now frame (isPrevFrameAvailable)", i); return DVO_ERR_STATE; }
    const size_t P0 = g.P[0];
    if (c->active) {
        dim3 grid((unsigned)((P0 + 1023) / 1024), (unsigned)count);
        promote_masked_kernel<<<grid, 256, 0, c->stream>>>(g, c->prev_gray, c->prev_depth, c->gray[0], c->depth[0], first, c->active);
        c->launches++;
        DVO_CUDA(cudaGetLastError());
        return DVO_OK;
    }
    DVO_CUDA(cudaMemcpyAsync(c->gray[0] + lvl_at(g, 0, first), c->prev_gray + P0 * first, P0 * count, cudaMemcpyDeviceToDevice, c->stream));
    DVO_CUDA(cudaMemcpyAsync(c->depth[0] + lvl_at(g, 0, first), c->prev_depth + P0 * first, P0 * count * 2, cudaMemcpyDeviceToDevice, c->stream));
    return DVO_OK;
}
```

Baseline: 102,500.

## Replace iterative Canny hysteresis with union-find on row runs and drop edge bytes

The iterative strip-based hysteresis flood, which looped until no block changed, is replaced by a per-row bit-parallel flood followed by union-find over candidate runs in adjacent rows, with the parent table held in shared memory or a global fallback. The per-pixel edge byte image is no longer written during Canny; the edge bitmap is kept in scratch and expanded only on demand when a caller reads the edge buffer. This is meant to remove the data-dependent convergence loop and the byte-image stores, at the cost of atomics, a table that can spill to global memory, and a different shared-memory sizing that may lower occupancy.

```diff
diff --git a/rgbd_odometry_b200/csrc/capi.cu b/rgbd_odometry_b200/csrc/capi.cu
--- a/rgbd_odometry_b200/csrc/capi.cu
+++ b/rgbd_odometry_b200/csrc/capi.cu
@@ -102,6 +102,7 @@
     CREATE_CUDA(cudaGetDeviceProperties(&prop, cfg->device));
     c->sm_count = prop.multiProcessorCount;
     c->smem_optin = prop.sharedMemPerBlockOptin;
+    c->smem_per_sm = prop.sharedMemPerMultiprocessor; c->smem_reserved = prop.reservedSharedMemPerBlock;
     c->solve_shape = (cfg->max_batch <= c->sm_count) ? 512 : 256;
     if (const char* e = getenv("DVO_SOLVE_SHAPE")) { const int v = atoi(e); if (v == 256 || v == 512) c->solve_shape = v; }
     c->texel_mode = 1;
@@ -127,7 +128,7 @@
     const size_t T = (size_t)g.total, B = (size_t)g.Bmax;
     int rc = DVO_OK;
     auto A = [&](int r) { if (rc == DVO_OK) rc = r; };
-    for (int f = 0; f < 2; ++f) { A(dalloc(&c->gray[f], T)); A(dalloc(&c->edge[f], T)); }
+    for (int f = 0; f < 2; ++f) A(dalloc(&c->gray[f], T));
     A(dalloc(&c->depth[0], T));
     if (cfg->keep_now_depth) { A(dalloc(&c->depth[1], T)); A(dalloc(&c->prev_gray, B * (size_t)g.P[0])); A(dalloc(&c->prev_depth, B * (size_t)g.P[0])); }
     c->now_valid = (unsigned char*)calloc(B, 1); c->prev_valid = (unsigned char*)calloc(B, 1);
@@ -138,8 +139,9 @@
     A(dalloc(&c->pose0, B * 12)); A(dalloc(&c->pose, B * 12)); A(dalloc(&c->info, B));
     if (cfg->trace_iters > 0) A(dalloc(&c->trace, B * g.L * cfg->trace_iters * DVO_TRACE_DOUBLES));
     A(dalloc(&c->energy, B * g.L * DVO_ENERGY_ITERS));
-    canny_scratch_layout(g, c->bm_off, c->bm_words, &c->bitmap_scratch_words);
+    canny_scratch_layout(g, c->bm_off, c->bm_words, &c->bitmap_scratch_words, &c->uf_words);
     A(dalloc(&c->bitmap_scratch, c->bitmap_scratch_words * B * 2));
+    A(dalloc(&c->uf_table, c->uf_words * B * 2));
     if (rc != DVO_OK) { dvo_destroy(c); return rc; }
     CREATE_CUDA(cudaMemsetAsync(c->npts, 0, sizeof(int) * B * g.L, c->stream));
     CREATE_CUDA(cudaMemsetAsync(c->bitmap_scratch, 0, sizeof(uint32_t) * c->bitmap_scratch_words * B * 2, c->stream));
@@ -158,7 +160,7 @@
     if (!c) return DVO_OK;
     cudaSetDevice(c->cfg.device);
     if (c->own_stream) cudaStreamSynchronize(c->own_stream);
-    for (int f = 0; f < 2; ++f) { cudaFree(c->gray[f]); cudaFree(c->depth[f]); cudaFree(c->edge[f]); }
+    for (int f = 0; f < 2; ++f) { cudaFree(c->gray[f]); cudaFree(c->depth[f]); }
     cudaFree(c->gcol); cudaFree(c->d2); cudaFree(c->texel); cudaFree(c->tex8); cudaFree(c->ptsX); cudaFree(c->ptsY); cudaFree(c->ptsZ); cudaFree(c->ptsPix);
     cudaFree(c->npts); cudaFree(c->solve_order); cudaFree(c->seq_mask); cudaFree(c->seq_state); cudaFree(c->nedge); cudaFree(c->maxd2); cudaFree(c->pose0); cudaFree(c->pose); cudaFree(c->info);
     cudaFree(c->seq_rel); cudaFree(c->seq_kind); cudaFree(c->seq_reason); cudaFree(c->seq_glob); cudaFree(c->seq_cov); cudaFree(c->seq_gcov);
@@ -168,7 +170,7 @@
         if (c->seq_ev_ready[k]) cudaEventDestroy(c->seq_ev_ready[k]);
         if (c->seq_ev_free[k]) cudaEventDestroy(c->seq_ev_free[k]);
     }
-    cudaFree(c->trace); cudaFree(c->energy); cudaFree(c->bitmap_scratch); cudaFree(c->prev_gray); cudaFree(c->prev_depth); cudaFree(c->raw_bgr); cudaFree(c->raw_depth);
+    cudaFree(c->trace); cudaFree(c->energy); cudaFree(c->bitmap_scratch); cudaFree(c->uf_table); cudaFree(c->prev_gray); cudaFree(c->prev_depth); cudaFree(c->raw_bgr); cudaFree(c->raw_depth);
     free(c->now_valid); free(c->prev_valid);
     if (c->h_pose) cudaFreeHost(c->h_pose);
     if (c->h_info) cudaFreeHost(c->h_info);
@@ -697,7 +699,7 @@
     switch (which) {
         case DVO_BUF_GRAY: src = c->gray[frame] + o; es = 1; break;
         case DVO_BUF_DEPTH: if (!c->depth[frame]) { dvo_set_error("depth not stored for this frame"); return DVO_ERR_STATE; } src = c->depth[frame] + o; es = 2; break;
-        case DVO_BUF_EDGE: src = c->edge[frame] + o; es = 1; break;
+        case DVO_BUF_EDGE: es = 1; break;
         case DVO_BUF_D2: if (frame != DVO_FRAME_NOW) { dvo_set_error("d2 exists for the now frame only"); return DVO_ERR_ARG; } src = c->d2 + o; es = 4; break;
         case DVO_BUF_DTN: case DVO_BUF_GX: case DVO_BUF_GY:
             if (frame != DVO_FRAME_NOW) { dvo_set_error("DT exists for the now frame only"); return DVO_ERR_ARG; } src = c->texel ? c->texel + o : nullptr; es = 16; break;
@@ -709,6 +711,18 @@
         DVO_CUDA(cudaMalloc((void**)&d_tmp, P * 4));
         const int rc = launch_d2_from_texels(c, slot, level, d_tmp);
         cudaError_t ce = rc ? cudaSuccess : cudaMemcpyAsync(dst, d_tmp, P * 4, cudaMemcpyDeviceToHost, c->stream);
+        if (ce == cudaSuccess) ce = cudaStreamSynchronize(c->stream);
+        cudaFree(d_tmp);
+        if (rc) return rc;
+        DVO_CUDA(ce);
+        return DVO_OK;
+    }
+    if (which == DVO_BUF_EDGE) {
+        if (bytes < P) { dvo_set_error("dvo_get_level_buffer: destination too small"); return DVO_ERR_ARG; }
+        uint8_t* d_tmp = nullptr;
+        DVO_CUDA(cudaMalloc((void**)&d_tmp, P));
+        const int rc = launch_edge_bytes(c, slot, frame, level, d_tmp);
+        cudaError_t ce = rc ? cudaSuccess : cudaMemcpyAsync(dst, d_tmp, P, cudaMemcpyDeviceToHost, c->stream);
         if (ce == cudaSuccess) ce = cudaStreamSynchronize(c->stream);
         cudaFree(d_tmp);
         if (rc) return rc;
diff --git a/rgbd_odometry_b200/csrc/common.cuh b/rgbd_odometry_b200/csrc/common.cuh
--- a/rgbd_odometry_b200/csrc/common.cuh
+++ b/rgbd_odometry_b200/csrc/common.cuh
@@ -51,6 +51,7 @@
     int sm_count;
     int solve_shape;
     size_t smem_optin;
+    size_t smem_per_sm, smem_reserved;
 
     uint8_t* gray[2];
     uint16_t* depth[2];
@@ -58,7 +59,6 @@
     uint16_t* prev_depth;
     unsigned char* now_valid;
     unsigned char* prev_valid;
-    uint8_t* edge[2];
     uint16_t* gcol;
     int32_t* d2;
     float4* texel;
@@ -83,7 +83,9 @@
     size_t bitmap_scratch_words;
     long long bm_off[DVO_MAX_LEVELS];
     int bm_words[DVO_MAX_LEVELS];
-    size_t canny_smem_optin;
+    size_t canny_smem_optin[2];
+    unsigned* uf_table;
+    size_t uf_words;
 
     uint8_t* raw_bgr; float* raw_depth; size_t raw_capacity;
 
@@ -109,7 +111,8 @@
 
 int launch_pyramid(dvo_ctx* c, int first, int count, int frames_mask);
 int launch_canny(dvo_ctx* c, int first, int count, int frames_mask);
-void canny_scratch_layout(const PyrGeom& g, long long* bm_off, int* bm_words, size_t* words_per_image);
+void canny_scratch_layout(const PyrGeom& g, long long* bm_off, int* bm_words, size_t* words_per_image, size_t* uf_words);
+int launch_edge_bytes(dvo_ctx* c, int slot, int frame, int level, uint8_t* d_out);
 int launch_edt_rows(dvo_ctx* c, int first, int count);
 int launch_normgrad(dvo_ctx* c, int first, int count);
 int launch_pack(dvo_ctx* c, int first, int count);
diff --git a/rgbd_odometry_b200/csrc/preprocess.cu b/rgbd_odometry_b200/csrc/preprocess.cu
--- a/rgbd_odometry_b200/csrc/preprocess.cu
+++ b/rgbd_odometry_b200/csrc/preprocess.cu
@@ -136,7 +136,6 @@
 
 struct CannyArgs {
     const uint8_t* gray[2];
-    uint8_t* edge[2];
     const uint16_t* depth;
     uint16_t* gcol;
     float *X, *Y, *Z;
@@ -153,6 +152,9 @@
     int first;
     int bm_words;
     const unsigned char* active;
+    unsigned* uf;
+    long long uf_stride, uf_frame_stride;
+    unsigned uf_cap;
 };
 
 __device__ __forceinline__ void sobel3(const uint8_t* __restrict__ g, int w, int h, int y, int x, int& dx, int& dy) {
@@ -167,8 +169,6 @@
     int dx, dy; sobel3(g, w, h, y, x, dx, dy);
     return dx * dx + dy * dy;
 }
-
-__device__ __forceinline__ uint32_t expand4(uint32_t nib) { return (((nib & 0xFu) * 0x00204081u) & 0x01010101u) * 0xFFu; }
 
 __device__ __forceinline__ void row_sums(const uint8_t* __restrict__ grow, int w, int x, int lane, int& hs, int& hb) {
     const int v = (x < w) ? (int)grow[x] : 0;
@@ -388,16 +388,63 @@
 #define DVO_CANNY_STOP_AFTER 0
 #endif
 
-template <bool GLOBAL_BITMAPS> struct HystPtr { typedef volatile uint32_t* type; };
-template <> struct HystPtr<true> { typedef uint32_t* type; };
+__device__ __forceinline__ int row_next(const uint32_t* row, int x, uint32_t flip, int wd) {
+    int wx = x >> 5;
+    if (wx >= wd) return wd << 5;
+    uint32_t v = (row[wx] ^ flip) & (0xffffffffu << (x & 31));
+    while (v == 0u) {
+        if (++wx >= wd) return wd << 5;
+        v = row[wx] ^ flip;
+    }
+    return (wx << 5) + __ffs(v) - 1;
+}
+__device__ __forceinline__ bool row_bit(const uint32_t* row, int x) { return (row[x >> 5] >> (x & 31)) & 1u; }
+
+__device__ __forceinline__ unsigned uf_find(unsigned* P, unsigned x) {
+    volatile unsigned* V = P;
+    for (;;) {
+        const unsigned p = V[x];
+        if (p == x) return x;
+        const unsigned g = V[p];
+        if (g == p) return p;
+        V[x] = g;
+        x = g;
+    }
+}
+__device__ __forceinline__ void uf_unite(unsigned* P, unsigned a, unsigned b) {
+    for (;;) {
+        a = uf_find(P, a); b = uf_find(P, b);
+        if (a == b) return;
+        if (a > b) { const unsigned t = a; a = b; b = t; }
+        const unsigned old = atomicMin(P + b, a);
+        if (old == b) return;
+        b = old;
+    }
+}
+
+__device__ __forceinline__ int block_exclusive_scan(int v, int* s_scan) {
+    const int lane = threadIdx.x & 31, warp = threadIdx.x >> 5;
+    int incl = v;
+    for (int o = 1; o < 32; o <<= 1) { const int t = __shfl_up_sync(0xffffffffu, incl, o); if (lane >= o) incl += t; }
+    if (lane == 31) s_scan[warp] = incl;
+    __syncthreads();
+    if (threadIdx.x < 32) {
+        const int nwp = blockDim.x >> 5;
+        const int x = (lane < nwp) ? s_scan[lane] : 0;
+        int iv = x;
+        for (int o = 1; o < 32; o <<= 1) { const int t = __shfl_up_sync(0xffffffffu, iv, o); if (lane >= o) iv += t; }
+        if (lane < nwp) s_scan[lane] = iv - x;
+        if (lane == 31) s_scan[CANNY_MAX_WARPS] = iv;
+    }
+    __syncthreads();
+    return s_scan[warp] + incl - v;
+}
 
 template <bool GLOBAL_BITMAPS>
 __global__ void __launch_bounds__(768, 2) canny_kernel(CannyArgs a) {
     extern __shared__ uint32_t smem_u32[];
     __shared__ int s_scan[CANNY_MAX_WARPS + 1];
-    __shared__ int s_base;
     __shared__ unsigned s_cnt;
-    __shared__ unsigned char s_chg[2][768];
     const int T = blockDim.x;
     const int tid = threadIdx.x, lane = tid & 31, warp = tid >> 5;
 #if DVO_CANNY_INTERLEAVE
@@ -415,8 +462,10 @@
     const int w = a.w, h = a.h;
     const int wd = (w + 31) >> 5, pitch = wd + 2;
     const int nwords = a.bm_words;
-    uint32_t* C = GLOBAL_BITMAPS ? a.gscratch + (long long)b * a.gscratch_stride + (long long)frame * a.gscratch_frame_stride : smem_u32;
+    auto scratch = [&]() { return a.gscratch + (long long)b * a.gscratch_stride + (long long)frame * a.gscratch_frame_stride; };
+    uint32_t* C = GLOBAL_BITMAPS ? scratch() : smem_u32;
     uint32_t* E = C + nwords;
+    unsigned* rowbase = reinterpret_cast<unsigned*>(smem_u32) + (GLOBAL_BITMAPS ? 0 : 2 * nwords);
 
     if (GLOBAL_BITMAPS) {
         for (int i = tid; i < pitch; i += T) { C[i] = 0u; E[i] = 0u; C[(h + 1) * pitch + i] = 0u; E[(h + 1) * pitch + i] = 0u; }
@@ -424,7 +473,7 @@
             C[(y + 1) * pitch] = 0u; E[(y + 1) * pitch] = 0u; C[(y + 1) * pitch + wd + 1] = 0u; E[(y + 1) * pitch + wd + 1] = 0u;
         }
     } else {
-        const uint32_t* __restrict__ src = a.gscratch + (long long)b * a.gscratch_stride + (long long)frame * a.gscratch_frame_stride;
+        const uint32_t* __restrict__ src = scratch();
         if ((reinterpret_cast<uintptr_t>(src) & 15) == 0 && (nwords & 1) == 0) {
             const uint4* s4 = reinterpret_cast<const uint4*>(src); uint4* d4 = reinterpret_cast<uint4*>(C);
             for (int i = tid; i < (nwords >> 1); i += T) d4[i] = s4[i];
@@ -432,108 +481,116 @@
             for (int i = tid; i < 2 * nwords; i += T) C[i] = src[i];
         }
     }
-    if (tid == 0) { s_cnt = 0u; s_base = 0; }
+    if (tid == 0) s_cnt = 0u;
     __syncthreads();
 
 #if DVO_CANNY_STOP_AFTER == 1
     return;
 #endif
     {
-        const int Hs = max(1, min(h, min(T, 768) / wd));
-        const int Rh = (h + Hs - 1) / Hs;
-        const int items = wd * Hs;
-        const int sh = tid / wd, wx = tid - sh * wd;
-        const bool owner = tid < items;
-        const int ya = sh * Rh, yb = min(h, ya + Rh);
-        for (int i = tid; i < 2 * 768; i += T) (&s_chg[0][0])[i] = (i < 768) ? 1 : 0;
+        auto flood = [](uint32_t f, uint32_t c) {
+            const uint32_t up = ((c + f) ^ c) & c;
+            const uint32_t cr = __brev(c), fr = __brev(f);
+            return f | up | __brev(((cr + fr) ^ cr) & cr);
+        };
+        for (int y = tid; y < h; y += T) {
+            const uint32_t* cr = C + (y + 1) * pitch + 1;
+            uint32_t* er = E + (y + 1) * pitch + 1;
+            uint32_t carry = 0u;
+            for (int wx = 0; wx < wd; ++wx) {
+                const uint32_t c = cr[wx], s = er[wx] | (c & carry);
+                const uint32_t f = s ? flood(s, c) : 0u;
+                er[wx] = f; carry = f >> 31;
+            }
+            carry = 0u;
+            for (int wx = wd - 1; wx >= 0; --wx) {
+                const uint32_t c = cr[wx], f = er[wx], s = f | (c & (carry << 31));
+                const uint32_t g = (s != f) ? flood(s, c) : f;
+                if (g != f) er[wx] = g;
+                carry = g & 1u;
+            }
+            int n = 0;
+            uint32_t prev = 0u;
+            for (int wx = 0; wx < wd; ++wx) {
+                const uint32_t u = cr[wx] & ~er[wx];
+                n += __popc(u & ~((u << 1) | (prev >> 31)));
+                prev = u;
+            }
+            rowbase[y] = (unsigned)n;
+        }
         __syncthreads();
-        int cur = 0;
-        for (;;) {
-            int changed = 0;
-            bool active = false;
-            if (owner && ya < yb) {
-                for (int dsy = -1; dsy <= 1 && !active; ++dsy)
-                    for (int dwx = -1; dwx <= 1; ++dwx) {
-                        const int s2 = sh + dsy, w2 = wx + dwx;
-                        if (s2 >= 0 && s2 < Hs && w2 >= 0 && w2 < wd && s_chg[cur][s2 * wd + w2]) { active = true; break; }
-                    }
-            }
-            if (active) {
-                auto spread = [](uint32_t l, uint32_t c, uint32_t r) { return c | (c << 1) | (c >> 1) | (l >> 31) | (r << 31); };
-                auto flood = [](uint32_t f, uint32_t c) {
-                    const uint32_t up = ((c + f) ^ c) & c;
-                    const uint32_t cr = __brev(c), fr = __brev(f);
-                    return f | up | __brev(((cr + fr) ^ cr) & cr);
-                };
-                typename HystPtr<GLOBAL_BITMAPS>::type Ev = E;
-                const uint32_t* Cv = C;
-                {
-                    int idx = (ya + 1) * pitch + wx + 1;
-                    uint32_t sp = spread(Ev[idx - pitch - 1], Ev[idx - pitch], Ev[idx - pitch + 1]);
-                    uint32_t el = Ev[idx - 1], ec = Ev[idx], er = Ev[idx + 1];
-                    for (int y = ya; y < yb; ++y, idx += pitch) {
-                        const uint32_t nl = Ev[idx + pitch - 1], nc = Ev[idx + pitch], nr = Ev[idx + pitch + 1];
-                        const uint32_t c = Cv[idx];
-                        uint32_t f = ec;
-                        if (c != 0u && ec != c) {
-                            f = flood(ec | (c & (sp | spread(el, ec, er) | spread(nl, nc, nr))), c);
-                            if (f != ec) { Ev[idx] = f; changed = 1; }
-                        }
-                        sp = spread(el, f, er); el = nl; ec = nc; er = nr;
-                    }
+        const int per = (h + T - 1) / T;
+        const int r0 = min(h, tid * per), r1 = min(h, r0 + per);
+        int mine = 0;
+        for (int y = r0; y < r1; ++y) mine += (int)rowbase[y];
+        unsigned off = 1u + (unsigned)block_exclusive_scan(mine, s_scan);
+        for (int y = r0; y < r1; ++y) { const unsigned n = rowbase[y]; rowbase[y] = off; off += n; }
+        const unsigned nodes = 1u + (unsigned)s_scan[CANNY_MAX_WARPS];
+        if (tid == 0) rowbase[h] = nodes;
+        unsigned* P = (nodes <= a.uf_cap) ? rowbase + h + 1
+                                          : a.uf + (long long)b * a.uf_stride + (long long)frame * a.uf_frame_stride;
+        for (unsigned i = tid; i < nodes; i += T) P[i] = i;
+        __syncthreads();
+
+        for (int y = tid + 1; y < h; y += T) {
+            unsigned nr = rowbase[y], nq = rowbase[y - 1];
+            if (rowbase[y + 1] == nq) continue;
+            const int ir = (y + 1) * pitch + 1, iq = ir - pitch;
+            int qa = row_next(C + iq, 0, 0u, wd), qb = 0;
+            unsigned qn = 0u;
+            auto load_q = [&]() { if (qa < w) { qb = row_next(C + iq, qa + 1, ~0u, wd) - 1; qn = row_bit(E + iq, qa) ? 0u : nq++; } };
+            load_q();
+            for (int ra = row_next(C + ir, 0, 0u, wd); ra < w && qa < w; ) {
+                const int rb = row_next(C + ir, ra + 1, ~0u, wd) - 1;
+                const unsigned rn = row_bit(E + ir, ra) ? 0u : nr++;
+                while (qa < w && qb < ra - 1) { qa = row_next(C + iq, qb + 2, 0u, wd); load_q(); }
+                while (qa < w && qa <= rb + 1) {
+                    if (rn | qn) uf_unite(P, rn, qn);
+                    if (qb > rb) break;
+                    qa = row_next(C + iq, qb + 2, 0u, wd); load_q();
                 }
-                {
-                    int idx = yb * pitch + wx + 1;
-                    uint32_t sp = spread(Ev[idx + pitch - 1], Ev[idx + pitch], Ev[idx + pitch + 1]);
-                    uint32_t el = Ev[idx - 1], ec = Ev[idx], er = Ev[idx + 1];
-                    for (int y = yb - 1; y >= ya; --y, idx -= pitch) {
-                        const uint32_t nl = Ev[idx - pitch - 1], nc = Ev[idx - pitch], nr = Ev[idx - pitch + 1];
-                        const uint32_t c = Cv[idx];
-                        uint32_t f = ec;
-                        if (c != 0u && ec != c) {
-                            f = flood(ec | (c & (sp | spread(el, ec, er) | spread(nl, nc, nr))), c);
-                            if (f != ec) { Ev[idx] = f; changed = 1; }
-                        }
-                        sp = spread(el, f, er); el = nl; ec = nc; er = nr;
-                    }
+                ra = row_next(C + ir, rb + 2, 0u, wd);
+            }
+        }
+        __syncthreads();
+
+        unsigned cnt = 0;
+        for (int y = tid; y < h; y += T) {
+            const uint32_t* cr = C + (y + 1) * pitch + 1;
+            uint32_t* er = E + (y + 1) * pitch + 1;
+            unsigned n = rowbase[y];
+            const unsigned n_end = rowbase[y + 1];
+            for (int ra = row_next(cr, 0, 0u, wd); n < n_end; ) {
+                const int rb = row_next(cr, ra + 1, ~0u, wd) - 1;
+                if (!row_bit(er, ra)) {
+                    if (uf_find(P, n) == 0u)
+                        for (int wx = ra >> 5; wx <= (rb >> 5); ++wx)
+                            er[wx] |= (0xffffffffu << max(ra - (wx << 5), 0)) & (0xffffffffu >> max((wx << 5) + 31 - rb, 0));
+                    ++n;
                 }
-            }
-            if (owner) s_chg[cur ^ 1][tid] = (unsigned char)changed;
-            cur ^= 1;
-            if (!__syncthreads_or(changed)) break;
-        }
+                ra = row_next(cr, rb + 2, 0u, wd);
+            }
+            for (int wx = 0; wx < wd; ++wx) cnt += __popc(er[wx]);
+        }
+        for (int o = 16; o > 0; o >>= 1) cnt += __shfl_down_sync(0xffffffffu, cnt, o);
+        if (lane == 0 && cnt) atomicAdd(&s_cnt, cnt);
+        __syncthreads();
     }
 
 #if DVO_CANNY_STOP_AFTER == 2
     return;
 #endif
     const int nw = h * wd;
-    {
-        uint8_t* eo = a.edge[frame] + (long long)b * a.P;
-        unsigned cnt = 0;
-        const bool vec_ok = (w % 16 == 0) && ((reinterpret_cast<uintptr_t>(eo) & 15) == 0);
-        for (int q = tid; q < nw; q += T) {
-            const int y = q / wd, wx = q - y * wd;
-            const uint32_t e = E[(y + 1) * pitch + wx + 1];
-            cnt += __popc(e);
-            const int x0 = wx << 5;
-            if (vec_ok && x0 + 32 <= w) {
-                uint4 v0, v1;
-                v0.x = expand4(e); v0.y = expand4(e >> 4); v0.z = expand4(e >> 8); v0.w = expand4(e >> 12);
-                v1.x = expand4(e >> 16); v1.y = expand4(e >> 20); v1.z = expand4(e >> 24); v1.w = expand4(e >> 28);
-                uint4* dst = reinterpret_cast<uint4*>(eo + (long long)y * w + x0);
-                dst[0] = v0; dst[1] = v1;
-            } else {
-                for (int i = 0; i < 32 && x0 + i < w; ++i) eo[(long long)y * w + x0 + i] = ((e >> i) & 1u) ? 255 : 0;
-            }
-        }
-        for (int o = 16; o > 0; o >>= 1) cnt += __shfl_down_sync(0xffffffffu, cnt, o);
-        if (lane == 0 && cnt) atomicAdd(&s_cnt, cnt);
-    }
-
-#if DVO_CANNY_STOP_AFTER == 3
-    return;
-#endif
+    if (!GLOBAL_BITMAPS) {
+        uint32_t* dst = scratch() + nwords;
+        if ((reinterpret_cast<uintptr_t>(dst) & 15) == 0 && (nwords & 3) == 0) {
+            const uint4* s4 = reinterpret_cast<const uint4*>(E); uint4* d4 = reinterpret_cast<uint4*>(dst);
+            for (int i = tid; i < (nwords >> 2); i += T) d4[i] = s4[i];
+        } else {
+            for (int i = tid; i < nwords; i += T) dst[i] = E[i];
+        }
+    }
+    uint32_t* const S = C;
     if (do_points) {
         const uint16_t* __restrict__ dep = a.depth + (long long)b * a.P;
         for (int q = tid; q < nw; q += T) {
@@ -549,9 +606,12 @@
                 const unsigned d0 = dr[i0], d1 = dr[i1], d2 = dr[i2], d3 = dr[i3];
                 sel |= (d0 > 100u ? 1u << i0 : 0u) | (d1 > 100u ? 1u << i1 : 0u) | (d2 > 100u ? 1u << i2 : 0u) | (d3 > 100u ? 1u << i3 : 0u);
             }
-            E[idx] = sel;
-        }
-    }
+            S[idx] = sel;
+        }
+    }
+#if DVO_CANNY_STOP_AFTER == 3
+    return;
+#endif
     __syncthreads();
     if (tid == 0) a.nedge[frame][(long long)b * a.L] = s_cnt;
 
@@ -559,8 +619,8 @@
     uint32_t* Et = C;
     if (do_cols) {
         const int nwarps = T >> 5;
-        for (int blk = warp; blk < hw * wd; blk += nwarps) {
-            const int wy = blk / wd, wx = blk - wy * wd;
+        int wy = warp / wd, wx = warp - wy * wd;
+        for (; wy < hw; wx += nwarps, wy += wx / wd, wx %= wd) {
             const int y = (wy << 5) + lane;
             const uint32_t word = (y < h) ? E[(y + 1) * pitch + wx + 1] : 0u;
             uint32_t mine = 0u;
@@ -608,24 +668,11 @@
         const int per = (nw + T - 1) / T;
         const int q0 = min(nw, tid * per), q1 = min(nw, q0 + per);
         int mycnt = 0;
-        for (int q = q0; q < q1; ++q) { const int y = q / wd, wx = q - y * wd; mycnt += __popc(E[(y + 1) * pitch + wx + 1]); }
-        int incl = mycnt;
-        for (int o = 1; o < 32; o <<= 1) { const int t = __shfl_up_sync(0xffffffffu, incl, o); if (lane >= o) incl += t; }
-        if (lane == 31) s_scan[warp] = incl;
-        __syncthreads();
-        if (tid < 32) {
-            const int nwp = T >> 5;
-            const int v = (tid < nwp) ? s_scan[tid] : 0;
-            int iv = v;
-            for (int o = 1; o < 32; o <<= 1) { const int t = __shfl_up_sync(0xffffffffu, iv, o); if (lane >= o) iv += t; }
-            if (tid < nwp) s_scan[tid] = iv - v;
-            if (tid == 31) s_scan[CANNY_MAX_WARPS] = iv;
-        }
-        __syncthreads();
-        int off = s_scan[warp] + (incl - mycnt);
+        for (int q = q0; q < q1; ++q) { const int y = q / wd, wx = q - y * wd; mycnt += __popc(S[(y + 1) * pitch + wx + 1]); }
+        int off = block_exclusive_scan(mycnt, s_scan);
         for (int q = q0; q < q1; ++q) {
             const int y = q / wd, wx = q - y * wd;
-            uint32_t v = E[(y + 1) * pitch + wx + 1];
+            uint32_t v = S[(y + 1) * pitch + wx + 1];
             const uint16_t* __restrict__ dr = dep + (long long)y * w;
             while (v) {
                 int xs[4], n = 0;
@@ -661,10 +708,11 @@
     return a > t ? a : t;
 }
 
-void canny_scratch_layout(const PyrGeom& g, long long* bm_off, int* bm_words, size_t* words_per_image) {
+void canny_scratch_layout(const PyrGeom& g, long long* bm_off, int* bm_words, size_t* words_per_image, size_t* uf_words) {
     long long o = 0;
     for (int l = 0; l < g.L; ++l) { bm_off[l] = o; bm_words[l] = canny_bitmap_words(g.w[l], g.h[l]); o += 2LL * ((bm_words[l] + 3) & ~3); }
     *words_per_image = (size_t)o;
+    *uf_words = (size_t)((g.w[0] + 1) / 2) * g.h[0] + 1;
 }
 
 int launch_canny(dvo_ctx* c, int first, int count, int frames_mask) {
@@ -698,11 +746,13 @@
     }
     for (int l = 0; l < g.L; ++l) {
         const int words = c->bm_words[l];
-        const size_t smem = (size_t)2 * words * sizeof(uint32_t);
-        const bool use_global = smem + 8192 > c->smem_optin;
-        const int wdl = (g.w[l] + 31) >> 5;
-        int strips = (CANNY_MAX_WARPS * 32) / wdl; if (strips > g.h[l]) strips = g.h[l]; if (strips < 1) strips = 1;
-        int threads = wdl * strips; if (threads < g.w[l]) threads = g.w[l];
+        const bool use_global = (size_t)2 * words * sizeof(uint32_t) + 8192 > c->smem_optin;
+        const long long fixed = (use_global ? 0LL : 8LL * words) + 4LL * (g.h[l] + 1);
+        long long room = (long long)(c->smem_per_sm / 2) - (long long)c->smem_reserved - 1024 - fixed;
+        if (room < 16384) room = (long long)c->smem_optin - 1024 - fixed;
+        const unsigned uf_cap = (unsigned)std::max(0LL, std::min(room / 4, (long long)words));
+        const size_t smem = (size_t)fixed + 4 * (size_t)uf_cap;
+        int threads = std::max(std::max(g.w[l], g.h[l]), ((g.w[l] + 31) >> 5) * g.h[l]);
         int warps = (threads + 31) / 32; if (warps > CANNY_MAX_WARPS) warps = CANNY_MAX_WARPS; if (warps < 4) warps = 4;
         {
             static int cap[DVO_MAX_LEVELS] = {-1};
@@ -720,7 +770,7 @@
         const int T = warps * 32;
         CannyArgs a;
         for (int f = 0; f < 2; ++f) {
-            a.gray[f] = c->gray[f] + g.off[l]; a.edge[f] = c->edge[f] + g.off[l];
+            a.gray[f] = c->gray[f] + g.off[l];
             a.nedge[f] = c->nedge + (size_t)f * g.Bmax * g.L + l;
         }
         a.depth = c->depth[0] ? c->depth[0] + g.off[l] : nullptr;
@@ -738,15 +788,14 @@
         a.gscratch_stride = slot_stride;
         a.gscratch_frame_stride = frame_stride;
         a.first = first; a.bm_words = words; a.active = c->active;
+        a.uf = c->uf_table; a.uf_stride = (long long)c->uf_words; a.uf_frame_stride = (long long)c->uf_words * g.Bmax; a.uf_cap = uf_cap;
         const int nblocks = both ? 2 * count : count;
-        if (use_global) canny_kernel<true><<<nblocks, T, 0, c->stream>>>(a);
-        else {
-            if (smem > 48 * 1024 && smem > c->canny_smem_optin) {
-                DVO_CUDA(cudaFuncSetAttribute(canny_kernel<false>, cudaFuncAttributeMaxDynamicSharedMemorySize, (int)smem));
-                c->canny_smem_optin = smem;
-            }
-            canny_kernel<false><<<nblocks, T, smem, c->stream>>>(a);
-        }
+        if (smem > 48 * 1024 && smem > c->canny_smem_optin[use_global]) {
+            DVO_CUDA(cudaFuncSetAttribute(use_global ? canny_kernel<true> : canny_kernel<false>, cudaFuncAttributeMaxDynamicSharedMemorySize, (int)smem));
+            c->canny_smem_optin[use_global] = smem;
+        }
+        if (use_global) canny_kernel<true><<<nblocks, T, smem, c->stream>>>(a);
+        else canny_kernel<false><<<nblocks, T, smem, c->stream>>>(a);
         c->launches++;
     }
     DVO_CUDA(cudaGetLastError());
@@ -1338,6 +1387,22 @@
     return DVO_OK;
 }
 
+__global__ void __launch_bounds__(256) edge_bytes_kernel(const uint32_t* __restrict__ E, uint8_t* __restrict__ out, int w, int h) {
+    const int i = blockIdx.x * 256 + threadIdx.x;
+    if (i >= w * h) return;
+    const int y = i / w, x = i - y * w, pitch = ((w + 31) >> 5) + 2;
+    out[i] = ((E[(y + 1) * pitch + (x >> 5) + 1] >> (x & 31)) & 1u) ? 255 : 0;
+}
+
+int launch_edge_bytes(dvo_ctx* c, int slot, int frame, int level, uint8_t* d_out) {
+    const PyrGeom& g = c->geom;
+    const uint32_t* E = c->bitmap_scratch + (size_t)c->bitmap_scratch_words * ((size_t)frame * g.Bmax + slot) + c->bm_off[level] + c->bm_words[level];
+    edge_bytes_kernel<<<(g.P[level] + 255) / 256, 256, 0, c->stream>>>(E, d_out, g.w[level], g.h[level]);
+    c->launches++;
+    DVO_CUDA(cudaGetLastError());
+    return DVO_OK;
+}
+
 __global__ void __launch_bounds__(256) promote_masked_kernel(PyrGeom g, const uint8_t* __restrict__ prev_gray, const uint16_t* __restrict__ prev_depth,
                                                              uint8_t* __restrict__ gray, uint16_t* __restrict__ depth, int first,
                                                              const unsigned char* __restrict__ active) {
```

Measured after the change: 86030 (median of 6 runs). -16.1%, worse.
